# ravenprotocol/ravnest

Measured on AMD Instinct MI355X. Metric: samples/sec (whole node), BERT-base MLM pretraining, higher is better.
Workload: dtype bf16; 1 GPU; model=bert-base, global_batch=128, seq_len=512, parallelism=dp1, reduce_factor=4, optimizer=fused_adam

## Files before the change

ravnest_amd/csrc/bindings.cpp:

```cpp
#include <torch/extension.h>

#include <vector>

std::vector<at::Tensor> layernorm_fwd(at::Tensor x, at::Tensor w,
                                      at::Tensor b, double eps);
std::vector<at::Tensor> layernorm_bwd(at::Tensor dy, at::Tensor x,
                                      at::Tensor w, at::Tensor mean,
                                      at::Tensor rstd);
std::vector<at::Tensor> layernorm_add_fwd(at::Tensor a, at::Tensor b,
                                          at::Tensor w, at::Tensor bias,
                                          double eps);
at::Tensor bias_gelu_fwd(at::Tensor x, at::Tensor bias);
at::Tensor bias_gelu_bwd(at::Tensor dy, at::Tensor x, at::Tensor bias);
at::Tensor colsum_bf16(at::Tensor x);
std::vector<at::Tensor> bias_gelu_bwd_db(at::Tensor dy, at::Tensor x,
                                         at::Tensor bias);
std::vector<at::Tensor> batchnorm_fwd(at::Tensor x, at::Tensor w,
                                      at::Tensor b, at::Tensor running_mean,
                                      at::Tensor running_var, bool training,
                                      double momentum, double eps);
std::vector<at::Tensor> batchnorm_bwd(at::Tensor dy, at::Tensor x,
                                      at::Tensor w, at::Tensor mean,
                                      at::Tensor rstd);
at::Tensor conv2d_fwd(at::Tensor x, at::Tensor w,
                      c10::optional<at::Tensor> bias, long st, long pad,
                      bool relu);
at::Tensor conv2d_dgrad(at::Tensor dy, at::Tensor w, long N, long H,
                        long W, long st, long pad);
at::Tensor conv2d_wgrad(at::Tensor dy, at::Tensor x, long R, long S,
                        long st, long pad);
std::vector<at::Tensor> mx_quant(at::Tensor x);
std::vector<at::Tensor> gemm_nt_bf16(at::Tensor A2, at::Tensor B,
                                     c10::optional<at::Tensor> bias,
                                     int64_t epi);
at::Tensor gemm_wgrad_bf16(at::Tensor dy, at::Tensor x);
at::Tensor mx_gemm(at::Tensor x, at::Tensor xs, at::Tensor w,
                   at::Tensor ws);
at::Tensor mx_gemm2(at::Tensor xq, at::Tensor xs, at::Tensor wq,
                    at::Tensor ws);
at::Tensor mx_scale_probe(at::Tensor a, at::Tensor b, at::Tensor sa,
                          at::Tensor sb);
at::Tensor softmax_fwd(at::Tensor x);
at::Tensor softmax_bwd(at::Tensor dy, at::Tensor y);
std::vector<at::Tensor> maxpool2d_fwd(at::Tensor x, long K, long S, long P);
at::Tensor maxpool2d_bwd(at::Tensor dy, at::Tensor idx, long H, long W,
                         long K, long S, long P);
at::Tensor avgpool2d_fwd(at::Tensor x, long K, long S, long P,
                         bool include_pad);
at::Tensor avgpool2d_bwd(at::Tensor dy, long H, long W, long K, long S,
                         long P, bool include_pad);
at::Tensor global_avgpool_fwd(at::Tensor x);
at::Tensor global_avgpool_bwd(at::Tensor dy, long H, long W);
std::vector<at::Tensor> emb2_ln_fwd(at::Tensor ids, at::Tensor word,
                                    at::Tensor pos, at::Tensor w,
                                    at::Tensor b, double eps);
at::Tensor emb2_add_fwd(at::Tensor ids, at::Tensor word, at::Tensor pos);
std::vector<at::Tensor> emb2_bwd(at::Tensor dx, at::Tensor ids, long V,
                                 long P);
std::vector<at::Tensor> dropout_fwd(at::Tensor x, double p, int64_t seed,
                                    c10::optional<at::Tensor> seed_buf);
at::Tensor dropout_bwd(at::Tensor dy, at::Tensor mask, double p);
std::vector<at::Tensor> dropout_add_ln_fwd(at::Tensor z, at::Tensor a,
                                           at::Tensor w, at::Tensor bias,
                                           double eps, double p, int64_t seed,
                                           c10::optional<at::Tensor> seed_buf);
std::vector<at::Tensor> dropout_add_ln_bwd(at::Tensor dy, at::Tensor s,
                                           at::Tensor w, at::Tensor mean,
                                           at::Tensor rstd,
                                           at::Tensor maskbits, double p);
std::vector<at::Tensor> ce_fwd(at::Tensor logits, at::Tensor targets,
                               int64_t ignore_index);
at::Tensor ce_bwd(at::Tensor logits, at::Tensor targets, at::Tensor lse,
                  at::Tensor gscale, int64_t ignore_index);
std::tuple<at::Tensor, long, long> adam_build_table(
    std::vector<at::Tensor> ps, std::vector<at::Tensor> gs,
    std::vector<at::Tensor> ms, std::vector<at::Tensor> vs,
    std::vector<at::Tensor> masters);
std::tuple<at::Tensor, long, long> grad_build_table(
    std::vector<at::Tensor> gs);
void grad_sqnorm(at::Tensor table, long nchunks, long esize,
                 at::Tensor partials, long offset);
void grad_norm_finalize(at::Tensor partials, long n, at::Tensor stats,
                        double max_norm,
                        c10::optional<at::Tensor> max_norm_buf);
void scale_mt(at::Tensor table, long nchunks, long esize, at::Tensor gstats);
void fused_adam_graph(at::Tensor table, long nchunks, long esize,
                      at::Tensor lr_buf, double b1, double b2, double eps,
                      double wd, at::Tensor step_buf,
                      c10::optional<at::Tensor> gstats);
void fused_adam_table(at::Tensor table, long nchunks, long esize, double lr,
                      double b1, double b2, double eps, double wd, double bc1,
                      double bc2, c10::optional<at::Tensor> gstats);
void fused_sgd_table(at::Tensor table, long nchunks, long esize, double lr,
                     double momentum, double wd, bool nesterov,
                     c10::optional<at::Tensor> gstats);
void fused_lamb_table(at::Tensor table, long nchunks, long esize,
                      long ntensors, double lr, double b1, double b2,
                      double eps, double wd, double bc1, double bc2,
                      double clamp_trust, c10::optional<at::Tensor> gstats);
void fused_adam(std::vector<at::Tensor> ps, std::vector<at::Tensor> gs,
                std::vector<at::Tensor> ms, std::vector<at::Tensor> vs,
                std::vector<at::Tensor> masters, double lr, double b1,
                double b2, double eps, double wd, double bc1, double bc2);
void fused_sgd(std::vector<at::Tensor> ps, std::vector<at::Tensor> gs,
               std::vector<at::Tensor> bufs, std::vector<at::Tensor> masters,
               double lr, double momentum, double wd, bool nesterov);
void fused_lamb(std::vector<at::Tensor> ps, std::vector<at::Tensor> gs,
                std::vector<at::Tensor> ms, std::vector<at::Tensor> vs,
                std::vector<at::Tensor> masters, double lr, double b1,
                double b2, double eps, double wd, double bc1, double bc2,
                double clamp_trust);
void fused_copy(std::vector<at::Tensor> srcs, std::vector<at::Tensor> dsts);
std::vector<at::Tensor> attn_fwd(at::Tensor q, at::Tensor k, at::Tensor v,
                                 at::Tensor mask, bool causal, double scale);
std::vector<at::Tensor> attn_bwd(at::Tensor q, at::Tensor k, at::Tensor v,
                                 at::Tensor o, at::Tensor dout,
                                 at::Tensor lse, at::Tensor mask, bool causal,
                                 double scale);
std::vector<at::Tensor> attn_fwd_qkv(at::Tensor qkv, at::Tensor mask,
                                     bool causal, double scale,
                                     double pdrop, int64_t dseed,
                                     c10::optional<at::Tensor> seed_buf);
at::Tensor attn_bwd_qkv(at::Tensor qkv, at::Tensor o, at::Tensor dout,
                        at::Tensor lse, at::Tensor mask, bool causal,
                        double scale, double pdrop,
                        c10::optional<at::Tensor> mbits);
at::Tensor mfma_probe(at::Tensor a, at::Tensor b);
at::Tensor tr16_probe();
at::Tensor mfma_mx_probe(at::Tensor a, at::Tensor b, int64_t sa, int64_t sb);

PYBIND11_MODULE(TORCH_EXTENSION_NAME, m) {
  m.def("layernorm_fwd", &layernorm_fwd, "fused LayerNorm fwd (CDNA4)");
  m.def("layernorm_bwd", &layernorm_bwd, "fused LayerNorm bwd (CDNA4)");
  m.def("layernorm_add_fwd", &layernorm_add_fwd,
        "fused residual-add + LayerNorm fwd");
  m.def("bias_gelu_fwd", &bias_gelu_fwd, "fused bias+GELU fwd");
  m.def("bias_gelu_bwd", &bias_gelu_bwd, "fused bias+GELU bwd");
  m.def("colsum_bf16", &colsum_bf16, "column sum bf16 -> fp32");
  m.def("bias_gelu_bwd_db", &bias_gelu_bwd_db,
        "fused bias+GELU bwd with in-pass bias-grad column reduction");
  m.def("batchnorm_fwd", &batchnorm_fwd, "fused BatchNorm2d fwd (NCHW)");
  m.def("batchnorm_bwd", &batchnorm_bwd, "fused BatchNorm2d bwd (NCHW)");
  m.def("dropout_fwd", &dropout_fwd, "philox dropout fwd (replayable)",
        py::arg("x"), py::arg("p"), py::arg("seed"),
        py::arg("seed_buf") = py::none());
  m.def("dropout_bwd", &dropout_bwd, "dropout bwd");
  m.def("dropout_add_ln_fwd", &dropout_add_ln_fwd,
        "fused dropout + residual add + LayerNorm fwd (bf16, bit mask)",
        py::arg("z"), py::arg("a"), py::arg("w"), py::arg("bias"),
        py::arg("eps"), py::arg("p"), py::arg("seed"),
        py::arg("seed_buf") = py::none());
  m.def("dropout_add_ln_bwd", &dropout_add_ln_bwd,
        "fused dropout + residual add + LayerNorm bwd: dx, dz, dw, db");
  m.def("conv2d_fwd", &conv2d_fwd,
        "implicit-GEMM MFMA conv fwd (bf16 NCHW)", py::arg("x"),
        py::arg("w"), py::arg("bias") = py::none(), py::arg("st") = 1,
        py::arg("pad") = 0, py::arg("relu") = false);
  m.def("conv2d_dgrad", &conv2d_dgrad, "implicit-GEMM MFMA conv dgrad");
  m.def("conv2d_wgrad", &conv2d_wgrad, "implicit-GEMM MFMA conv wgrad");
  m.def("gemm_nt_bf16", &gemm_nt_bf16,
        "bf16 MFMA GEMM x @ W^T (256^2 8-phase, fused bias/GELU epilogue)",
        py::arg("a"), py::arg("b"), py::arg("bias") = py::none(),
        py::arg("epi") = 0);
  m.def("gemm_wgrad_bf16", &gemm_wgrad_bf16,
        "split-K wgrad dW = dy^T @ x (tr16 transpose reads, fp32 atomics)");
  m.def("mx_quant", &mx_quant,
        "bf16 -> MX fp8 (e4m3 + per-32 e8m0 scales)");
  m.def("mx_gemm", &mx_gemm, "MX fp8 GEMM: x @ W^T, 32x32x64 scaled MFMA");
  m.def("mx_gemm2", &mx_gemm2,
        "LDS-staged MX fp8 GEMM (256^2 4-phase, scaled 32x32x64 MFMA)");
  m.def("mx_scale_probe", &mx_scale_probe,
        "per-lane scale-byte semantics probe");
  m.def("softmax_fwd", &softmax_fwd, "standalone softmax fwd (last dim)");
  m.def("softmax_bwd", &softmax_bwd, "standalone softmax bwd");
  m.def("maxpool2d_fwd", &maxpool2d_fwd, "MaxPool2d fwd (+argmax idx)");
  m.def("maxpool2d_bwd", &maxpool2d_bwd, "MaxPool2d bwd (gather)");
  m.def("avgpool2d_fwd", &avgpool2d_fwd, "AvgPool2d fwd");
  m.def("avgpool2d_bwd", &avgpool2d_bwd, "AvgPool2d bwd");
  m.def("global_avgpool_fwd", &global_avgpool_fwd,
        "global (adaptive 1x1) avg pool fwd");
  m.def("global_avgpool_bwd", &global_avgpool_bwd, "global avg pool bwd");
  m.def("emb2_ln_fwd", &emb2_ln_fwd,
        "fused word+pos embedding gather + LayerNorm fwd");
  m.def("emb2_add_fwd", &emb2_add_fwd, "fused word+pos embedding gather");
  m.def("emb2_bwd", &emb2_bwd,
        "embedding bwd: dword scatter-add + dpos batch reduction");
  m.def("ce_fwd", &ce_fwd, "fused softmax cross-entropy fwd");
  m.def("ce_bwd", &ce_bwd, "fused softmax cross-entropy bwd");
  m.def("fused_adam", &fused_adam, "multi-tensor Adam");
  m.def("adam_build_table", &adam_build_table,
        "prebuild the device chunk table (graph-capturable Adam)");
  m.def("fused_adam_graph", &fused_adam_graph,
        "multi-tensor Adam with device lr/step buffers (hipGraph mode)",
        py::arg("table"), py::arg("nchunks"), py::arg("esize"),
        py::arg("lr_buf"), py::arg("b1"), py::arg("b2"), py::arg("eps"),
        py::arg("wd"), py::arg("step_buf"), py::arg("gstats") = py::none());
  m.def("mt_build_table", &adam_build_table,
        "prebuild the device chunk table (any fused optimizer)");
  m.def("grad_build_table", &grad_build_table,
        "grads-only device chunk table (clip_grad_norm_)");
  m.def("grad_sqnorm", &grad_sqnorm,
        "multi-tensor per-chunk sum of squared grads -> partials");
  m.def("grad_norm_finalize", &grad_norm_finalize,
        "partials -> [norm, clip coefficient, non-finite count]",
        py::arg("partials"), py::arg("n"), py::arg("stats"),
        py::arg("max_norm"), py::arg("max_norm_buf") = py::none());
  m.def("scale_mt", &scale_mt, "multi-tensor in-place g *= stats[1]");
  m.def("fused_adam_table", &fused_adam_table,
        "multi-tensor Adam from a prebuilt table (+ clip coefficient)",
        py::arg("table"), py::arg("nchunks"), py::arg("esize"),
        py::arg("lr"), py::arg("b1"), py::arg("b2"), py::arg("eps"),
        py::arg("wd"), py::arg("bc1"), py::arg("bc2"),
        py::arg("gstats") = py::none());
  m.def("fused_sgd_table", &fused_sgd_table,
        "multi-tensor SGD from a prebuilt table (+ clip coefficient)",
        py::arg("table"), py::arg("nchunks"), py::arg("esize"),
        py::arg("lr"), py::arg("momentum"), py::arg("wd"),
        py::arg("nesterov"), py::arg("gstats") = py::none());
  m.def("fused_lamb_table", &fused_lamb_table,
        "multi-tensor LAMB from a prebuilt table (+ clip coefficient)",
        py::arg("table"), py::arg("nchunks"), py::arg("esize"),
        py::arg("ntensors"), py::arg("lr"), py::arg("b1"), py::arg("b2"),
        py::arg("eps"), py::arg("wd"), py::arg("bc1"), py::arg("bc2"),
        py::arg("clamp_trust"), py::arg("gstats") = py::none());
  m.def("fused_sgd", &fused_sgd, "multi-tensor SGD+momentum");
  m.def("fused_lamb", &fused_lamb, "multi-tensor LAMB");
  m.def("fused_copy", &fused_copy, "multi-tensor device copy");
  m.def("attn_fwd", &attn_fwd, "flash attention fwd (bf16, MFMA)");
  m.def("attn_bwd", &attn_bwd, "flash attention bwd (bf16, MFMA, D=64)");
  m.def("attn_fwd_qkv", &attn_fwd_qkv,
        py::arg("qkv"), py::arg("mask"), py::arg("causal"),
        py::arg("scale"), py::arg("pdrop") = 0.0, py::arg("dseed") = 0,
        py::arg("seed_buf") = py::none(),
        "flash attention fwd, packed (B,S,3,H,D) qkv -> (B,S,H,D)");
  m.def("attn_bwd_qkv", &attn_bwd_qkv,
        py::arg("qkv"), py::arg("o"), py::arg("dout"), py::arg("lse"),
        py::arg("mask"), py::arg("causal"), py::arg("scale"),
        py::arg("pdrop") = 0.0, py::arg("mbits") = py::none(),
        "flash attention bwd, packed qkv -> dqkv");
  m.def("mfma_probe", &mfma_probe, "32x32x16 bf16 MFMA layout probe");
  m.def("tr16_probe", &tr16_probe, "ds_read_b64_tr_b16 mapping probe");
  m.def("mfma_mx_probe", &mfma_mx_probe,
        "32x32x64 MX-scaled fp8 MFMA layout probe");
}
```

ravnest_amd/csrc/ce_loss.hip:

```cpp
#include <torch/extension.h>
#include <ATen/hip/HIPContext.h>

#include "common.h"

namespace {

template <typename T>
DEVINL float ld(const T* p);
template <>
DEVINL float ld<bf16_t>(const bf16_t* p) { return bf2f(*p); }
template <>
DEVINL float ld<float>(const float* p) { return *p; }

DEVINL void ms_merge(float& m, float& s, float m2, float s2) {
  const float mn = fmaxf(m, m2);
  if (mn == -INFINITY) { m = mn; return; }
  s = s * __expf(m - mn) + s2 * __expf(m2 - mn);
  m = mn;
}

template <typename T>
__global__ void ce_fwd_kernel(const T* __restrict__ logits,
                              const long* __restrict__ targets,
                              float* __restrict__ lse_out,
                              float* __restrict__ loss_accum,
                              int* __restrict__ valid_accum, int V, long N,
                              long ignore_index) {
  __shared__ float scratch_m[16];
  __shared__ float scratch_s[16];
  const long row = blockIdx.x;
  if (row >= N) return;
  const T* lr = logits + row * V;
  const long tgt = targets[row];

  float m = -INFINITY, s = 0.f;
  if constexpr (sizeof(T) == 2) {
    const int nv = V >> 3;
    for (int g = threadIdx.x; g < nv; g += blockDim.x) {
      const bf16x8 v8 = *reinterpret_cast<const bf16x8*>(lr + g * 8);
      float vals[8], vmax = -INFINITY;
#pragma unroll
      for (int j = 0; j < 8; ++j) {
        vals[j] = us2f((unsigned short)v8[j]);
        vmax = fmaxf(vmax, vals[j]);
      }
      float ls = 0.f;
#pragma unroll
      for (int j = 0; j < 8; ++j) ls += __expf(vals[j] - vmax);
      if (vmax > m) {
        s = s * __expf(m - vmax) + ls;
        m = vmax;
      } else {
        s += ls * __expf(vmax - m);
      }
    }
    for (int i = (nv << 3) + threadIdx.x; i < V; i += blockDim.x) {
      const float v = ld(lr + i);
      if (v > m) {
        s = s * __expf(m - v) + 1.f;
        m = v;
      } else {
        s += __expf(v - m);
      }
    }
  } else {
    for (int i = threadIdx.x; i < V; i += blockDim.x) {
      const float v = ld(lr + i);
      if (v > m) {
        s = s * __expf(m - v) + 1.f;
        m = v;
      } else {
        s += __expf(v - m);
      }
    }
  }
#pragma unroll
  for (int off = 32; off > 0; off >>= 1) {
    float m2 = __shfl_down(m, off, WAVE);
    float s2 = __shfl_down(s, off, WAVE);
    ms_merge(m, s, m2, s2);
  }
  {
    const int lane = threadIdx.x & (WAVE - 1);
    const int wid = threadIdx.x / WAVE;
    const int nw = (blockDim.x + WAVE - 1) / WAVE;
    if (lane == 0) {
      scratch_m[wid] = m;
      scratch_s[wid] = s;
    }
    __syncthreads();
    if (wid == 0) {
      m = (threadIdx.x < nw) ? scratch_m[threadIdx.x] : -INFINITY;
      s = (threadIdx.x < nw) ? scratch_s[threadIdx.x] : 0.f;
#pragma unroll
      for (int off = 32; off > 0; off >>= 1) {
        float m2 = __shfl_down(m, off, WAVE);
        float s2 = __shfl_down(s, off, WAVE);
        ms_merge(m, s, m2, s2);
      }
      if (threadIdx.x == 0) {
        scratch_m[0] = m;
        scratch_s[0] = s;
      }
    }
    __syncthreads();
    m = scratch_m[0];
    s = scratch_s[0];
  }
  const float lse = m + __logf(s);

  if (threadIdx.x == 0) {
    lse_out[row] = lse;
    if (tgt != ignore_index) {
      atomicAdd(loss_accum, lse - ld(lr + tgt));
      atomicAdd(valid_accum, 1);
    }
  }
}

template <typename T>
__global__ void ce_bwd_kernel(const T* __restrict__ logits,
                              const long* __restrict__ targets,
                              const float* __restrict__ lse,
                              const float* __restrict__ gscale,
                              T* __restrict__ dlogits, int V, long N,
                              long ignore_index) {
  const long row = blockIdx.x;
  if (row >= N) return;
  const T* lr = logits + row * V;
  T* dr = dlogits + row * V;
  const long tgt = targets[row];
  const float g = gscale[0];
  const float l = lse[row];
  if (tgt == ignore_index) {
    for (int i = threadIdx.x; i < V; i += blockDim.x) {
      if constexpr (sizeof(T) == 2)
        dr[i] = f2bf(0.f);
      else
        dr[i] = 0.f;
    }
    return;
  }
  if constexpr (sizeof(T) == 2) {
    const int nv = V >> 3;
    for (int gi = threadIdx.x; gi < nv; gi += blockDim.x) {
      const bf16x8 v8 = *reinterpret_cast<const bf16x8*>(lr + gi * 8);
      bf16x8 o;
#pragma unroll
      for (int j = 0; j < 8; ++j) {
        const int i = gi * 8 + j;
        float p = __expf(us2f((unsigned short)v8[j]) - l);
        o[j] = (short)f2us((p - (i == (int)tgt ? 1.f : 0.f)) * g);
      }
      *reinterpret_cast<bf16x8*>(dr + gi * 8) = o;
    }
    for (int i = (nv << 3) + threadIdx.x; i < V; i += blockDim.x) {
      float p = __expf(ld(lr + i) - l);
      dr[i] = f2bf((p - (i == (int)tgt ? 1.f : 0.f)) * g);
    }
  } else {
    for (int i = threadIdx.x; i < V; i += blockDim.x) {
      float p = __expf(ld(lr + i) - l);
      dr[i] = (p - (i == (int)tgt ? 1.f : 0.f)) * g;
    }
  }
}

}

std::vector<at::Tensor> ce_fwd(at::Tensor logits, at::Tensor targets,
                               int64_t ignore_index) {
  TORCH_CHECK(logits.is_cuda() && logits.is_contiguous());
  TORCH_CHECK(logits.dim() == 2);
  TORCH_CHECK(targets.scalar_type() == at::kLong);
  const long N = logits.size(0);
  const int V = logits.size(1);
  auto lse = at::empty({N}, logits.options().dtype(at::kFloat));
  auto loss = at::zeros({1}, logits.options().dtype(at::kFloat));
  auto nvalid = at::zeros({1}, logits.options().dtype(at::kInt));
  auto stream = c10::hip::getCurrentHIPStreamMasqueradingAsCUDA().stream();
  dim3 block(256);
  dim3 grid(N);
  if (logits.scalar_type() == at::kBFloat16) {
    hipLaunchKernelGGL((ce_fwd_kernel<bf16_t>), grid, block, 0, stream,
                       reinterpret_cast<const bf16_t*>(logits.data_ptr()),
                       targets.data_ptr<long>(), lse.data_ptr<float>(),
                       loss.data_ptr<float>(), nvalid.data_ptr<int>(), V, N,
                       ignore_index);
  } else {
    hipLaunchKernelGGL((ce_fwd_kernel<float>), grid, block, 0, stream,
                       logits.data_ptr<float>(), targets.data_ptr<long>(),
                       lse.data_ptr<float>(), loss.data_ptr<float>(),
                       nvalid.data_ptr<int>(), V, N, ignore_index);
  }
  HIP_CHECK_LAST();
  return {loss.squeeze(0), lse, nvalid.squeeze(0)};
}

at::Tensor ce_bwd(at::Tensor logits, at::Tensor targets, at::Tensor lse,
                  at::Tensor gscale, int64_t ignore_index) {
  TORCH_CHECK(logits.is_cuda() && logits.is_contiguous());
  const long N = logits.size(0);
  const int V = logits.size(1);
  auto dlogits = at::empty_like(logits);
  auto gs = gscale.to(at::kFloat).reshape({1}).contiguous();
  auto stream = c10::hip::getCurrentHIPStreamMasqueradingAsCUDA().stream();
  dim3 block(256);
  dim3 grid(N);
  if (logits.scalar_type() == at::kBFloat16) {
    hipLaunchKernelGGL((ce_bwd_kernel<bf16_t>), grid, block, 0, stream,
                       reinterpret_cast<const bf16_t*>(logits.data_ptr()),
                       targets.data_ptr<long>(), lse.data_ptr<float>(),
                       gs.data_ptr<float>(),
                       reinterpret_cast<bf16_t*>(dlogits.data_ptr()), V, N,
                       ignore_index);
  } else {
    hipLaunchKernelGGL((ce_bwd_kernel<float>), grid, block, 0, stream,
                       logits.data_ptr<float>(), targets.data_ptr<long>(),
                       lse.data_ptr<float>(), gs.data_ptr<float>(),
                       dlogits.data_ptr<float>(), V, N, ignore_index);
  }
  HIP_CHECK_LAST();
  return dlogits;
}
```

ravnest_amd/csrc/gemm.hip:

```cpp
#include <torch/extension.h>
#include <ATen/hip/HIPContext.h>

#include "common.h"

typedef __bf16 bf16x8v __attribute__((ext_vector_type(8)));
typedef unsigned short u16x4 __attribute__((ext_vector_type(4)));

#define LDS_V8(p)                                            \
  *reinterpret_cast<__attribute__((address_space(3))) const  \
                        bf16x8v*>(                           \
      (__attribute__((address_space(3))) const void*)(p))

namespace {

constexpr int BM = 256, BN = 256, BK = 64;
constexpr int HALF_BYTES = 128 * BK * 2;
constexpr int TILE_BYTES = 2 * HALF_BYTES;
constexpr int BUF_BYTES = 2 * TILE_BYTES;

DEVINL float gelu_f(float x) {
  const float k = 0.7978845608028654f;
  const float t = __expf(2.f * k * (x + 0.044715f * x * x * x));
  return x * t / (t + 1.f);
}

DEVINL unsigned stage_off(long ld, long gR0, long gRmax, int i) {
  const int tid = threadIdx.x;
  const int p = i * 8192 + (tid >> 6) * 1024 + (tid & 63) * 16;
  const int rr = p >> 7;
  const int cb = (p & 127) ^ (((p >> 8) & 7) << 4);
  long g = gR0 + rr;
  if (g > gRmax) g = gRmax;
  return (unsigned)(g * ld * 2 + cb);
}

DEVINL int frag_off(int rr, int kc, int lane) {
  const int cb = ((lane >> 4) << 4) + (kc << 6);
  const int p = (rr << 7) + cb;
  return p ^ (((p >> 8) & 7) << 4);
}

template <int EPI>
__global__ __launch_bounds__(512, 2) void gemm_nt_kernel(
    const bf16_t* __restrict__ A, const bf16_t* __restrict__ B,
    const bf16_t* __restrict__ bias, bf16_t* __restrict__ C,
    bf16_t* __restrict__ H, long M, long N, long K, int MT, int NTb,
    int tpb) {
  __shared__ char smem[2 * BUF_BYTES];

  const int nwg = MT * NTb;
  int bid = blockIdx.x, wg;
  if ((nwg & 7) == 0) {
    wg = (bid & 7) * (nwg >> 3) + (bid >> 3);
  } else {
    const int q = nwg >> 3, r = nwg & 7, x = bid & 7, lin = bid >> 3;
    wg = (x < r ? x * (q + 1) : r * (q + 1) + (x - r) * q) + lin;
  }
  constexpr int GM = 8;
  const int group = wg / (GM * NTb);
  const int lid = wg % (GM * NTb);
  const int gsz = min(GM, MT - group * GM);
  const int bm = group * GM + lid % gsz;
  const int bn0 = (lid / gsz) * tpb;

  const int tid = threadIdx.x;
  const int lane = tid & 63;
  const int wid = tid >> 6;
  const int wm = wid >> 2, wn = wid & 3;

  const long mBase = (long)bm * BM;
  const long nBase = (long)bn0 * BN;
  const int nKT = (int)(K / BK);
  const unsigned SJ = (unsigned)(BN * K * 2);

  unsigned sp[4][2];
  unsigned capB[2];
#pragma unroll
  for (int i = 0; i < 2; ++i) {
    sp[0][i] = stage_off(K, mBase, M - 1, i);
    sp[1][i] = stage_off(K, mBase + 128, M - 1, i);
    sp[2][i] = stage_off(K, nBase, N - 1, i);
    sp[3][i] = stage_off(K, nBase + 128, N - 1, i);
    capB[i] = stage_off(K, 0, 0, i) + (unsigned)((N - 1) * K * 2);
  }
  const int slo[4] = {0, HALF_BYTES, TILE_BYTES, TILE_BYTES + HALF_BYTES};
  const int wbase = (threadIdx.x >> 6) * 1024;
  auto stage = [&](int jj, int tt, int kind) {
    if (jj >= tpb) {
      jj = tpb - 1;
      tt = nKT - 1;
    }
    const unsigned off = (unsigned)tt * (BK * 2);
    const int b = (jj * nKT + tt) & 1;
    char* const lb = smem + b * BUF_BYTES + slo[kind] + wbase;
    const char* const base =
        reinterpret_cast<const char*>(kind >= 2 ? B : A);
#pragma unroll
    for (int i = 0; i < 2; ++i) {
      unsigned o = sp[kind][i];
      if (kind >= 2) {
        o += (unsigned)jj * SJ;
        if (o > capB[i]) o = capB[i];
      }
      __builtin_amdgcn_global_load_lds(
          (const __attribute__((address_space(1))) void*)(base + o + off),
          (__attribute__((address_space(3))) void*)(lb + i * 8192),
          16, 0, 0);
    }
  };
  auto norm = [&](int j, int t, int dt, int& jj, int& tt) {
    tt = t + dt;
    jj = j;
    if (tt >= nKT) {
      tt -= nKT;
      ++jj;
    }
  };

  stage(0, 0, 0); stage(0, 0, 2); stage(0, 0, 3); stage(0, 0, 1);
  stage(0, 1, 2); stage(0, 1, 3); stage(0, 1, 0);
  asm volatile("s_waitcnt vmcnt(6)" ::: "memory");
  __builtin_amdgcn_s_barrier();

  const int l15 = lane & 15;

  bf16x8v aF[4][2], bF[4][2];

  for (int j = 0; j < tpb; ++j) {
  f32x4 acc[8][4];
#pragma unroll
  for (int m = 0; m < 8; ++m)
#pragma unroll
    for (int n = 0; n < 4; ++n) acc[m][n] = f32x4{0.f, 0.f, 0.f, 0.f};

  for (int t = 0; t < nKT; ++t) {
    const int b = (j * nKT + t) & 1;
    int jj, tt;
    char* const aH0 = smem + b * BUF_BYTES + wm * HALF_BYTES;
    char* const bH =
        smem + b * BUF_BYTES + TILE_BYTES + (wn >> 1) * HALF_BYTES;
    const int bRow0 = (wn & 1) * 64;

#pragma unroll
    for (int nf = 0; nf < 2; ++nf)
#pragma unroll
      for (int kc = 0; kc < 2; ++kc)
        bF[nf][kc] = LDS_V8(bH + frag_off(bRow0 + nf * 16 + l15, kc, lane));
#pragma unroll
    for (int mf = 0; mf < 4; ++mf)
#pragma unroll
      for (int kc = 0; kc < 2; ++kc)
        aF[mf][kc] = LDS_V8(aH0 + frag_off(mf * 16 + l15, kc, lane));
    norm(j, t, 1, jj, tt);
    stage(jj, tt, 1);
    asm volatile("s_waitcnt lgkmcnt(8)" ::: "memory");
    __builtin_amdgcn_s_setprio(1);
#pragma unroll
    for (int mf = 0; mf < 4; ++mf)
#pragma unroll
      for (int nf = 0; nf < 2; ++nf)
#pragma unroll
        for (int kc = 0; kc < 2; ++kc)
          acc[mf][nf] = __builtin_amdgcn_mfma_f32_16x16x32_bf16(
              bF[nf][kc], aF[mf][kc], acc[mf][nf], 0, 0, 0);
    __builtin_amdgcn_s_setprio(0);
    __builtin_amdgcn_s_barrier();

#pragma unroll
    for (int nf = 2; nf < 4; ++nf)
#pragma unroll
      for (int kc = 0; kc < 2; ++kc)
        bF[nf][kc] = LDS_V8(bH + frag_off(bRow0 + nf * 16 + l15, kc, lane));
    __builtin_amdgcn_s_setprio(1);
#pragma unroll
    for (int mf = 0; mf < 4; ++mf)
#pragma unroll
      for (int nf = 2; nf < 4; ++nf)
#pragma unroll
        for (int kc = 0; kc < 2; ++kc)
          acc[mf][nf] = __builtin_amdgcn_mfma_f32_16x16x32_bf16(
              bF[nf][kc], aF[mf][kc], acc[mf][nf], 0, 0, 0);
    __builtin_amdgcn_s_setprio(0);
    __builtin_amdgcn_s_barrier();

#pragma unroll
    for (int mf = 0; mf < 4; ++mf)
#pragma unroll
      for (int kc = 0; kc < 2; ++kc)
        aF[mf][kc] = LDS_V8(aH0 + frag_off(64 + mf * 16 + l15, kc, lane));
    norm(j, t, 2, jj, tt);
    stage(jj, tt, 2);
    __builtin_amdgcn_s_setprio(1);
#pragma unroll
    for (int mf = 0; mf < 4; ++mf)
#pragma unroll
      for (int nf = 0; nf < 2; ++nf)
#pragma unroll
        for (int kc = 0; kc < 2; ++kc)
          acc[4 + mf][nf] = __builtin_amdgcn_mfma_f32_16x16x32_bf16(
              bF[nf][kc], aF[mf][kc], acc[4 + mf][nf], 0, 0, 0);
    __builtin_amdgcn_s_setprio(0);
    __builtin_amdgcn_s_barrier();

    stage(jj, tt, 3);
    stage(jj, tt, 0);
    __builtin_amdgcn_s_setprio(1);
#pragma unroll
    for (int mf = 0; mf < 4; ++mf)
#pragma unroll
      for (int nf = 2; nf < 4; ++nf)
#pragma unroll
        for (int kc = 0; kc < 2; ++kc)
          acc[4 + mf][nf] = __builtin_amdgcn_mfma_f32_16x16x32_bf16(
              bF[nf][kc], aF[mf][kc], acc[4 + mf][nf], 0, 0, 0);
    __builtin_amdgcn_s_setprio(0);
    asm volatile("s_waitcnt vmcnt(6)" ::: "memory");
    __builtin_amdgcn_s_barrier();
  }

  const long mRow0 = mBase + wm * 128 + l15;
  const long nCol0 = nBase + (long)j * BN + wn * 64 + ((lane >> 4) << 2);
  auto epilogue = [&](auto interior) {
#pragma unroll
    for (int mf = 0; mf < 8; ++mf) {
      const long m = mRow0 + mf * 16;
      if constexpr (!interior.value) {
        if (m >= M) continue;
      }
#pragma unroll
      for (int nf = 0; nf < 4; ++nf) {
        const long n = nCol0 + nf * 16;
        bool full = true;
        if constexpr (!interior.value) {
          if (n >= N) continue;
          full = (n + 4 <= N);
        }
        float v0 = acc[mf][nf][0], v1 = acc[mf][nf][1];
        float v2 = acc[mf][nf][2], v3 = acc[mf][nf][3];
        if (EPI >= 1) {
          if (full) {
            const u16x4 bb = *reinterpret_cast<const u16x4*>(bias + n);
            v0 += us2f(bb[0]); v1 += us2f(bb[1]);
            v2 += us2f(bb[2]); v3 += us2f(bb[3]);
          } else {
            v0 += bf2f(bias[n]);
            if (n + 1 < N) v1 += bf2f(bias[n + 1]);
            if (n + 2 < N) v2 += bf2f(bias[n + 2]);
          }
        }
        if (EPI == 2) {
          u16x4 h{f2us(v0), f2us(v1), f2us(v2), f2us(v3)};
          if (full) {
            *reinterpret_cast<u16x4*>(H + m * N + n) = h;
          } else {
            for (int v = 0; v < 4; ++v)
              if (n + v < N) H[m * N + n + v] = f2bf(us2f(h[v]));
          }
          v0 = gelu_f(v0); v1 = gelu_f(v1);
          v2 = gelu_f(v2); v3 = gelu_f(v3);
        }
        const u16x4 o{f2us(v0), f2us(v1), f2us(v2), f2us(v3)};
        if (full) {
          *reinterpret_cast<u16x4*>(C + m * N + n) = o;
        } else {
          for (int v = 0; v < 4; ++v)
            if (n + v < N) C[m * N + n + v] = f2bf(us2f(o[v]));
        }
      }
    }
  };
  if (mRow0 + 7 * 16 < M && nCol0 + 3 * 16 + 4 <= N)
    epilogue(std::true_type{});
  else
    epilogue(std::false_type{});
  }
  asm volatile("s_waitcnt vmcnt(0)" ::: "memory");
}

}

std::vector<at::Tensor> gemm_nt_bf16(at::Tensor A2, at::Tensor B,
                                     c10::optional<at::Tensor> bias,
                                     int64_t epi) {
  TORCH_CHECK(A2.is_cuda() && A2.scalar_type() == at::kBFloat16 &&
              A2.is_contiguous() && A2.dim() == 2);
  TORCH_CHECK(B.is_cuda() && B.scalar_type() == at::kBFloat16 &&
              B.is_contiguous() && B.dim() == 2);
  const long M = A2.size(0), K = A2.size(1), N = B.size(0);
  TORCH_CHECK(B.size(1) == K, "gemm_nt_bf16: K mismatch");
  TORCH_CHECK(K % BK == 0 && K >= 2 * BK,
              "gemm_nt_bf16: K % 64 == 0 and K >= 128 required");
  TORCH_CHECK(A2.numel() * 2 < (1ll << 32) && B.numel() * 2 < (1ll << 32),
              "gemm_nt_bf16: operands must be < 4 GiB (32-bit staging "
              "offsets)");
  TORCH_CHECK(epi == 0 || bias.has_value(), "bias required for epi>=1");
  const bf16_t* bp = nullptr;
  if (bias.has_value()) {
    TORCH_CHECK(bias->is_contiguous() &&
                bias->scalar_type() == at::kBFloat16 && bias->numel() == N);
    bp = reinterpret_cast<const bf16_t*>(bias->data_ptr());
  }
  auto C = at::empty({M, N}, A2.options());
  at::Tensor Hp;
  bf16_t* hp = nullptr;
  if (epi == 2) {
    Hp = at::empty({M, N}, A2.options());
    hp = reinterpret_cast<bf16_t*>(Hp.data_ptr());
  }
  const int MT = (int)((M + BM - 1) / BM), NT = (int)((N + BN - 1) / BN);
  int tpb = 1;
  for (int cand : {8, 6, 4, 3, 2}) {
    if (NT % cand == 0 && (long)MT * (NT / cand) >= 512) {
      tpb = cand;
      break;
    }
  }
  const int NTb = NT / tpb;
  auto stream = c10::hip::getCurrentHIPStreamMasqueradingAsCUDA().stream();
  dim3 grid((unsigned)(MT * NTb)), block(512);
  auto* a = reinterpret_cast<const bf16_t*>(A2.data_ptr());
  auto* b = reinterpret_cast<const bf16_t*>(B.data_ptr());
  auto* c = reinterpret_cast<bf16_t*>(C.data_ptr());
  switch (epi) {
    case 0:
      hipLaunchKernelGGL((gemm_nt_kernel<0>), grid, block, 0, stream, a, b,
                         bp, c, hp, M, N, K, MT, NTb, tpb);
      break;
    case 1:
      hipLaunchKernelGGL((gemm_nt_kernel<1>), grid, block, 0, stream, a, b,
                         bp, c, hp, M, N, K, MT, NTb, tpb);
      break;
    default:
      hipLaunchKernelGGL((gemm_nt_kernel<2>), grid, block, 0, stream, a, b,
                         bp, c, hp, M, N, K, MT, NTb, tpb);
  }
  HIP_CHECK_LAST();
  if (epi == 2) return {C, Hp};
  return {C};
}
```

ravnest_amd/csrc/gemm_wgrad.hip:

```cpp
#include <torch/extension.h>
#include <ATen/hip/HIPContext.h>

#include "common.h"

typedef __bf16 bf16x4v __attribute__((ext_vector_type(4)));
typedef __bf16 bf16x8v __attribute__((ext_vector_type(8)));
typedef short s16x8 __attribute__((ext_vector_type(8)));

#define DS_TR16(p)                                   \
  __builtin_amdgcn_ds_read_tr16_b64_v4bf16(          \
      (__attribute__((address_space(3))) bf16x4v*)(  \
          (__attribute__((address_space(3))) void*)(p)))

namespace {

constexpr int BN = 128, BK = 128, BM = 64;
constexpr int ROWB = 256;
constexpr int DY_BYTES = BM * ROWB;
constexpr int PAIR_BYTES = 2 * DY_BYTES;

DEVINL int swz(int row, int cb) { return cb ^ ((row & 7) << 5); }

template <bool TAIL>
__global__ __launch_bounds__(256, 2) void wgrad_kernel(
    const bf16_t* __restrict__ DY, const bf16_t* __restrict__ X,
    float* __restrict__ WS, long M, long N, long K, int NT, int KT,
    int splitk, long mTilesPer) {
  __shared__ char smem[2 * PAIR_BYTES];

  const int ntiles = NT * KT;
  const int nwg = ntiles * splitk;
  int bid = blockIdx.x, wg;
  if ((nwg & 7) == 0) {
    wg = (bid & 7) * (nwg >> 3) + (bid >> 3);
  } else {
    const int q = nwg >> 3, r = nwg & 7, x = bid & 7, lin = bid >> 3;
    wg = (x < r ? x * (q + 1) : r * (q + 1) + (x - r) * q) + lin;
  }
  const int tile = wg / splitk, slice = wg % splitk;
  const int bn = tile % NT, bk = tile / NT;
  const long n0 = (long)bn * BN, k0 = (long)bk * BK;
  const bool is_tail = (n0 + BN > N) || (k0 + BK > K);
  if (TAIL != is_tail) return;
  const long mt0 = slice * mTilesPer;
  const long mt1 = min(mt0 + mTilesPer, M / BM);
  if (mt0 >= mt1) return;

  const int tid = threadIdx.x;
  const int lane = tid & 63;
  const int wid = tid >> 6;
  const int wn = wid >> 1, wk = wid & 1;

  auto img = [&](int b, int op) {
    return smem + b * PAIR_BYTES + op * DY_BYTES;
  };

  long srcOff[8];
  int dstOff[8];
  int shiftv[8], validv[8];
#pragma unroll
  for (int i = 0; i < 8; ++i) {
    const int o = i * 4096 + wid * 1024 + lane * 16;
    const int op = o >= DY_BYTES;
    const int lo = op ? o - DY_BYTES : o;
    const int row = lo >> 8;
    const int cb = swz(row, lo & 255);
    const long cols = op ? K : N;
    const long cbase = op ? k0 : n0;
    long c = cbase + cb / 2;
    int sh = 0, va = 8;
    if (TAIL && c + 8 > cols) {
      const long cl = max(0l, cols - 8);
      sh = (int)(c - cl);
      va = (int)max(0l, min(8l, cols - c));
      c = cl;
    }
    srcOff[i] = ((long)row * cols + c) * 2;
    dstOff[i] = o;
    shiftv[i] = sh;
    validv[i] = va;
  }
  const long dyStep = (long)BM * N * 2, xStep = (long)BM * K * 2;

  auto stage_glds = [&](long mt, int b) {
#pragma unroll
    for (int i = 0; i < 8; ++i) {
      const int op = dstOff[i] >= DY_BYTES;
      const char* src = reinterpret_cast<const char*>(op ? X : DY) +
                        srcOff[i] + mt * (op ? xStep : dyStep);
      __builtin_amdgcn_global_load_lds(
          (const __attribute__((address_space(1))) void*)src,
          (__attribute__((address_space(3))) void*)(
              smem + b * PAIR_BYTES + (dstOff[i] - lane * 16)),
          16, 0, 0);
    }
  };

  s16x8 stg[8];
  auto issue_loads = [&](long mt) {
#pragma unroll
    for (int i = 0; i < 8; ++i) {
      const int op = dstOff[i] >= DY_BYTES;
      const char* s = reinterpret_cast<const char*>(op ? X : DY) +
                      srcOff[i] + mt * (op ? xStep : dyStep);
      stg[i] = *reinterpret_cast<const s16x8*>(s);
    }
  };
  auto write_stage = [&](int b) {
#pragma unroll
    for (int i = 0; i < 8; ++i) {
      s16x8 v = stg[i];
      if (shiftv[i] | (validv[i] ^ 8)) {
        s16x8 w;
        for (int j = 0; j < 8; ++j)
          w[j] = (j < validv[i]) ? v[j + shiftv[i]] : short(0);
        v = w;
      }
      *reinterpret_cast<s16x8*>(smem + b * PAIR_BYTES + dstOff[i]) = v;
    }
  };

  const int q4 = lane & 15, g = lane >> 4;
  auto tr_off = [&](int mc, int r, int colwin) {
    const int row = mc * 32 + g * 8 + r * 4 + (q4 >> 2);
    const int cb = (colwin + 4 * (q4 & 3)) * 2;
    return row * ROWB + swz(row, cb);
  };

  f32x4 acc[4][4];
#pragma unroll
  for (int a = 0; a < 4; ++a)
#pragma unroll
    for (int b = 0; b < 4; ++b) acc[a][b] = f32x4{0.f, 0.f, 0.f, 0.f};

  if (TAIL) {
    issue_loads(mt0);
    write_stage(0);
    __syncthreads();
  } else {
    stage_glds(mt0, 0);
    asm volatile("s_waitcnt vmcnt(0)" ::: "memory");
    __builtin_amdgcn_s_barrier();
  }

  for (long mt = mt0; mt < mt1; ++mt) {
    const int b = (int)((mt - mt0) & 1);
    if (mt + 1 < mt1) {
      if (TAIL)
        issue_loads(mt + 1);
      else
        stage_glds(mt + 1, b ^ 1);
    }

    bf16x8v aF[4][2], bF[4][2];
#pragma unroll
    for (int nf = 0; nf < 4; ++nf)
#pragma unroll
      for (int mc = 0; mc < 2; ++mc) {
        bf16x4v lo = DS_TR16(img(b, 0) + tr_off(mc, 0, wn * 64 + nf * 16));
        bf16x4v hi = DS_TR16(img(b, 0) + tr_off(mc, 1, wn * 64 + nf * 16));
        bf16x8v f;
        f[0] = lo[0]; f[1] = lo[1]; f[2] = lo[2]; f[3] = lo[3];
        f[4] = hi[0]; f[5] = hi[1]; f[6] = hi[2]; f[7] = hi[3];
        aF[nf][mc] = f;
      }
#pragma unroll
    for (int kf = 0; kf < 4; ++kf)
#pragma unroll
      for (int mc = 0; mc < 2; ++mc) {
        bf16x4v lo = DS_TR16(img(b, 1) + tr_off(mc, 0, wk * 64 + kf * 16));
        bf16x4v hi = DS_TR16(img(b, 1) + tr_off(mc, 1, wk * 64 + kf * 16));
        bf16x8v f;
        f[0] = lo[0]; f[1] = lo[1]; f[2] = lo[2]; f[3] = lo[3];
        f[4] = hi[0]; f[5] = hi[1]; f[6] = hi[2]; f[7] = hi[3];
        bF[kf][mc] = f;
      }

    __builtin_amdgcn_s_setprio(1);
#pragma unroll
    for (int mc = 0; mc < 2; ++mc)
#pragma unroll
      for (int nf = 0; nf < 4; ++nf)
#pragma unroll
        for (int kf = 0; kf < 4; ++kf)
          acc[nf][kf] = __builtin_amdgcn_mfma_f32_16x16x32_bf16(
              aF[nf][mc], bF[kf][mc], acc[nf][kf], 0, 0, 0);
    __builtin_amdgcn_s_setprio(0);

    if (TAIL) {
      if (mt + 1 < mt1) write_stage(b ^ 1);
      __syncthreads();
    } else {
      asm volatile("s_waitcnt vmcnt(0)" ::: "memory");
      __builtin_amdgcn_s_barrier();
    }
  }

#pragma unroll
  for (int nf = 0; nf < 4; ++nf)
#pragma unroll
    for (int kf = 0; kf < 4; ++kf) {
      const long k = k0 + wk * 64 + kf * 16 + (lane & 15);
      if (k >= K) continue;
#pragma unroll
      for (int v = 0; v < 4; ++v) {
        const long n = n0 + wn * 64 + nf * 16 + ((lane >> 4) << 2) + v;
        if (n < N) atomicAdd(WS + n * K + k, acc[nf][kf][v]);
      }
    }
}

}

at::Tensor gemm_wgrad_bf16(at::Tensor dy, at::Tensor x) {
  TORCH_CHECK(dy.is_cuda() && dy.scalar_type() == at::kBFloat16 &&
              dy.is_contiguous() && dy.dim() == 2);
  TORCH_CHECK(x.is_cuda() && x.scalar_type() == at::kBFloat16 &&
              x.is_contiguous() && x.dim() == 2);
  const long M = dy.size(0), N = dy.size(1), K = x.size(1);
  TORCH_CHECK(x.size(0) == M, "gemm_wgrad: M mismatch");
  TORCH_CHECK(M % BM == 0 && M >= 2 * BM,
              "gemm_wgrad: M % 64 == 0 and M >= 128 required");
  TORCH_CHECK(N >= 8 && K >= 8);
  auto ws = at::zeros({N, K}, dy.options().dtype(at::kFloat));
  const int NT = (int)((N + BN - 1) / BN), KT = (int)((K + BK - 1) / BK);
  const long mTiles = M / BM;
  const int ntiles = NT * KT;
  int splitk = (int)std::min<long>(
      mTiles, std::max<long>(1, (1536 + ntiles - 1) / ntiles));
  const long mTilesPer = (mTiles + splitk - 1) / splitk;
  splitk = (int)((mTiles + mTilesPer - 1) / mTilesPer);
  auto stream = c10::hip::getCurrentHIPStreamMasqueradingAsCUDA().stream();
  dim3 grid((unsigned)(ntiles * splitk)), block(256);
  const bool has_tail = (N % BN) || (K % BK);
  hipLaunchKernelGGL((wgrad_kernel<false>), grid, block, 0, stream,
                     reinterpret_cast<const bf16_t*>(dy.data_ptr()),
                     reinterpret_cast<const bf16_t*>(x.data_ptr()),
                     ws.data_ptr<float>(), M, N, K, NT, KT, splitk,
                     mTilesPer);
  if (has_tail)
    hipLaunchKernelGGL((wgrad_kernel<true>), grid, block, 0, stream,
                       reinterpret_cast<const bf16_t*>(dy.data_ptr()),
                       reinterpret_cast<const bf16_t*>(x.data_ptr()),
                       ws.data_ptr<float>(), M, N, K, NT, KT, splitk,
                       mTilesPer);
  HIP_CHECK_LAST();
  return ws;
}
```

ravnest_amd/engine/compute.py:

```python
from __future__ import annotations

import os
import threading
from dataclasses import dataclass

import torch

from ..utils import current_rng_states, restore_rng_states, trace_range


@dataclass
class _FpidRecord:
    version: int
    rng: dict
    args: list
    needs_grad: list
    recomputed_args: list | None = None
    recomputed_outputs: tuple | None = None


class ComputeEngine:
    def __init__(self, model: torch.nn.Module,
                 optimizer: torch.optim.Optimizer | None,
                 device: torch.device,
                 update_frequency: int = 1,
                 criterion=None,
                 loss_filename: str = "losses.txt",
                 amp_dtype: torch.dtype | None = None,
                 versioning: bool = True,
                 max_grad_norm: float | None = None):
        self.model = model
        self.optimizer = optimizer
        self.device = device
        self.update_frequency = max(1, update_frequency)
        self.criterion = criterion
        self.loss_filename = loss_filename
        self.amp_dtype = amp_dtype
        self.versioning = versioning
        self.max_grad_norm = max_grad_norm
        self._clip_external = False
        self._last_norm = None
        if max_grad_norm is not None and optimizer is not None:
            if hasattr(optimizer, "grad_norm_stats"):
                optimizer.max_grad_norm = max_grad_norm
            else:
                self._clip_external = True
        self._graph_step = None
        if (not versioning and device.type == "cuda"
                and self.update_frequency == 1 and criterion is not None
                and os.environ.get("RAVNEST_CUDA_GRAPH", "1") == "1"):
            from .graphstep import GraphedTrainStep
            self._graph_step = GraphedTrainStep(model, criterion, device,
                                                optimizer=optimizer)

        self.pre_step_hook = None

        self.current_version = 0
        self.version_to_param: dict[int, list[torch.Tensor]] = {}
        self.version_refs: dict[int, int] = {}
        self.fpids: dict[int, _FpidRecord] = {}
        self.n_backwards = 0
        self.file_loss = 0.0
        self._recompute_thread: threading.Thread | None = None
        self._lock = threading.Lock()

        self._params = list(self.model.parameters())
        self._snapshot_current()

    def _optimizer_step(self):
        if self._clip_external:
            from ..ops import clip_grad_norm_
            self._last_norm = clip_grad_norm_(self._params,
                                              self.max_grad_norm)
        self.optimizer.step()

    def last_grad_norm(self) -> float | None:
        if self.max_grad_norm is None or self.optimizer is None:
            return None
        if self._clip_external:
            return None if self._last_norm is None \
                else float(self._last_norm)
        stats = self.optimizer.grad_norm_stats()
        return None if stats is None else float(stats[0])

    def _autocast(self):
        if self.amp_dtype is not None and self.device.type == "cuda":
            return torch.autocast("cuda", dtype=self.amp_dtype)
        import contextlib
        return contextlib.nullcontext()

    def _snapshot_current(self):
        if not self.versioning:
            return
        snap = [torch.empty_like(p) for p in self._params]
        self._fast_copy([p.detach() for p in self._params], snap)
        self.version_to_param[self.current_version] = snap
        self.version_refs.setdefault(self.current_version, 0)

    def _fast_copy(self, srcs, dsts):
        if srcs and srcs[0].is_cuda:
            from ..ops import get_ext
            ext = get_ext(required=False)
            if ext is not None:
                ext.fused_copy(srcs, dsts)
                return
        for s, d in zip(srcs, dsts):
            d.copy_(s)

    def latest_state_snapshot(self) -> dict:
        with self._lock:
            if not self.versioning:
                return {"version": self.current_version,
                        "params": [p.detach().clone() for p in self._params]}
            return {
                "version": self.current_version,
                "params": [t.clone() for t in
                           self.version_to_param[self.current_version]],
            }

    def load_param_list(self, params: list[torch.Tensor]):
        with torch.no_grad():
            for p, src in zip(self._params, params):
                p.data.copy_(src.to(p.device))
        self.bump_version()

    def _release_version(self, v: int):
        self.version_refs[v] -= 1
        if self.version_refs[v] == 0 and v != self.current_version:
            del self.version_refs[v]
            del self.version_to_param[v]

    def bump_version(self):
        old = self.current_version
        self.current_version += 1
        if not self.versioning:
            return
        self._snapshot_current()
        if self.version_refs.get(old, 0) == 0:
            self.version_refs.pop(old, None)
            self.version_to_param.pop(old, None)

    def _swap_params_to(self, version: int):
        snap = self.version_to_param[version]
        for p, s in zip(self._params, snap):
            p.data = s

    def _restore_params(self):
        for p, orig in zip(self._params, self._orig_data):
            p.data = orig

    def forward(self, fpid: int, args: list, needs_grad: list) -> tuple:
        self.join_recompute()
        if not self.model.training:
            self.model.train()
        rng = current_rng_states(self.device)
        rec = _FpidRecord(version=self.current_version, rng=rng,
                          args=[a.detach().clone() if torch.is_tensor(a) else a
                                for a in args],
                          needs_grad=list(needs_grad))
        with torch.no_grad(), self._autocast(), trace_range(f"fwd:{fpid}"):
            out = self.model(*args)
        outputs = out if isinstance(out, tuple) else (out,)
        with self._lock:
            self.fpids[fpid] = rec
            self.version_refs[rec.version] = self.version_refs.get(rec.version, 0) + 1
        return outputs

    def _recompute(self, fpid: int):
        rec = self.fpids[fpid]
        if rec.recomputed_outputs is not None:
            return
        args = []
        for a, ng in zip(rec.args, rec.needs_grad):
            if torch.is_tensor(a) and a.is_floating_point():
                a = a.detach().clone().requires_grad_(True) if ng else a
            args.append(a)
        self._orig_data = [p.data for p in self._params]
        self._swap_params_to(rec.version)
        try:
            if not self.model.training:
                self.model.train()
            devices = [self.device] if self.device.type == "cuda" else []
            with torch.random.fork_rng(devices=devices):
                restore_rng_states(rec.rng, self.device)
                with self._autocast():
                    out = self.model(*args)
        finally:
            self._restore_params()
        rec.recomputed_outputs = out if isinstance(out, tuple) else (out,)
        rec.recomputed_args = args

    def join_recompute(self):
        t = self._recompute_thread
        if t is not None and t.is_alive():
            t.join()

    def backward(self, fpid: int, grads_by_out_idx: dict[int, torch.Tensor],
                 speculative_next: bool = True
                 ) -> tuple[list[torch.Tensor | None], bool]:
        self.join_recompute()
        rec = self.fpids[fpid]
        self._recompute(fpid)
        outs, grads = [], []
        for k, g in grads_by_out_idx.items():
            out = rec.recomputed_outputs[k]
            if out.grad_fn is None:
                continue
            outs.append(out)
            grads.append(g.to(out.dtype).to(out.device))
        if outs:
            with trace_range(f"bwd:{fpid}"):
                torch.autograd.backward(outs, grads)

        input_grads: list[torch.Tensor | None] = []
        for a, ng in zip(rec.recomputed_args, rec.needs_grad):
            if ng and torch.is_tensor(a):
                input_grads.append(a.grad if a.grad is not None
                                   else torch.zeros_like(a))
            else:
                input_grads.append(None)

        stepped = self._finish_backward(fpid, rec)
        if speculative_next and (fpid + 1) in self.fpids:
            self._recompute_thread = threading.Thread(
                target=self._recompute, args=(fpid + 1,), daemon=True)
            self._recompute_thread.start()
        return input_grads, stepped

    def _finish_backward(self, fpid: int, rec: _FpidRecord) -> bool:
        with self._lock:
            del self.fpids[fpid]
            self._release_version(rec.version)
        self.n_backwards += 1
        stepped = False
        if self.optimizer is not None and \
                self.n_backwards % self.update_frequency == 0:
            if self.pre_step_hook is not None:
                self.pre_step_hook()
            self._optimizer_step()
            self.optimizer.zero_grad(set_to_none=True)
            self.model.zero_grad(set_to_none=True)
            self.bump_version()
            stepped = True
        return stepped

    def find_loss(self, fpid: int, args: list, needs_grad: list, targets
                  ) -> tuple[list[torch.Tensor | None], bool, float]:
        self.join_recompute()
        if not self.model.training:
            self.model.train()
        if self._graph_step is not None and not any(needs_grad) and \
                self.amp_dtype is None:
            if self.pre_step_hook is not None:
                self.pre_step_hook()
            loss_t = self._graph_step.run(args, targets)
            if loss_t is not None:
                return self._finish_graphed_step(args, loss_t)
        if self._graph_step is not None and self._graph_step.graphs:
            self.model.zero_grad(set_to_none=True)
        live_args = []
        for a, ng in zip(args, needs_grad):
            if ng and torch.is_tensor(a) and a.is_floating_point():
                a = a.detach().clone().requires_grad_(True)
            live_args.append(a)
        with self._autocast():
            out = self.model(*live_args)
            loss = self.criterion(out, targets)
        loss.backward()
        loss_val = float(loss.detach())
        self.file_loss += loss_val

        input_grads: list[torch.Tensor | None] = []
        for a, ng in zip(live_args, needs_grad):
            if ng and torch.is_tensor(a):
                input_grads.append(a.grad if a.grad is not None
                                   else torch.zeros_like(a))
            else:
                input_grads.append(None)

        self.n_backwards += 1
        stepped = False
        if self.optimizer is not None and \
                self.n_backwards % self.update_frequency == 0:
            if self.pre_step_hook is not None:
                self.pre_step_hook()
            self._optimizer_step()
            self.optimizer.zero_grad(set_to_none=True)
            self.model.zero_grad(set_to_none=True)
            self.bump_version()
            stepped = True
            if self.loss_filename:
                with open(self.loss_filename, "a") as f:
                    f.write(f"{round(self.file_loss, 4)}\n")
            self.file_loss = 0.0
        return input_grads, stepped, loss_val

    def _finish_graphed_step(self, args, loss_t):
        self.n_backwards += 1
        stepped = False
        if self._graph_step.opt_captured:
            self.optimizer.bump_host_steps()
            stepped = True
        elif self.optimizer is not None:
            self._optimizer_step()
            stepped = True
        loss_val = float(loss_t)
        self.file_loss += loss_val
        if stepped:
            if self.loss_filename:
                with open(self.loss_filename, "a") as f:
                    f.write(f"{round(self.file_loss, 4)}\n")
            self.file_loss = 0.0
        return [None] * len(args), stepped, loss_val

    def no_grad_forward(self, args: list) -> tuple:
        self.join_recompute()
        self.model.eval()
        with torch.no_grad(), self._autocast():
            out = self.model(*args)
        return out if isinstance(out, tuple) else (out,)
```

ravnest_amd/engine/graphstep.py:

```python
from __future__ import annotations

import torch

from ..ops import rng


def _sig(tensors):
    return tuple((tuple(t.shape), t.dtype) for t in tensors)


class GraphedTrainStep:

    WARMUP = 3

    def __init__(self, model, criterion, device, optimizer=None):
        self.model = model
        self.criterion = criterion
        self.device = device
        import os
        use_opt = os.environ.get("RAVNEST_GRAPH_OPT", "0") == "1"
        self.optimizer = (optimizer if use_opt and
                          hasattr(optimizer, "graph_step") else None)
        self.opt_captured = False
        self.graphs = {}
        self.pool = None
        self.failed = False

    def run(self, args, targets):
        if self.failed or self.device.type != "cuda":
            return None
        if not all(torch.is_tensor(a) for a in args) or \
                not torch.is_tensor(targets):
            return None
        arg_ts = list(args)
        tgt_ts = [targets]
        key = (_sig(arg_ts), _sig(tgt_ts))
        entry = self.graphs.get(key)
        if entry is None:
            try:
                entry = self._capture(arg_ts, tgt_ts)
            except Exception:
                self.failed = True
                self.model.zero_grad(set_to_none=True)
                return None
            self.graphs[key] = entry
        graph, s_args, s_tgts, s_loss, grad_refs = entry
        if self.opt_captured:
            self.optimizer.sync_lr()
        for dst, src in zip(s_args, arg_ts):
            dst.copy_(src, non_blocking=True)
        for dst, src in zip(s_tgts, tgt_ts):
            dst.copy_(src, non_blocking=True)
        graph.replay()
        for param, gref in grad_refs:
            param.grad = gref
        return s_loss

    def _capture(self, arg_ts, tgt_ts):
        s_args = [t.clone() for t in arg_ts]
        s_tgts = [t.clone() for t in tgt_ts]
        self.model.train()
        rng.device_seed_counter(self.device)

        if self.optimizer is not None and not self.opt_captured:
            self.opt_captured = self.optimizer.enable_graph_capture(
                self.device)

        def step(with_opt=False, stable_grads=None):
            rng.bump_seed_counter(self.device)
            if with_opt:
                torch._foreach_zero_(stable_grads)
            out = self.model(*s_args)
            loss = self.criterion(out, s_tgts[0])
            loss.backward()
            if with_opt:
                self.optimizer.graph_step()
            return loss

        side = torch.cuda.Stream(self.device)
        side.wait_stream(torch.cuda.current_stream(self.device))
        with torch.cuda.stream(side):
            for _ in range(self.WARMUP):
                step()
        torch.cuda.current_stream(self.device).wait_stream(side)
        self.model.zero_grad(set_to_none=True)
        stable_grads = None
        if self.opt_captured:
            stable_grads = self.optimizer._graph.get("grads")
            if stable_grads is None:
                stable_grads = self.optimizer.build_graph_table()

        graph = torch.cuda.CUDAGraph()
        if self.pool is None:
            with torch.cuda.graph(graph):
                s_loss = step(self.opt_captured, stable_grads)
            self.pool = graph.pool()
        else:
            with torch.cuda.graph(graph, pool=self.pool):
                s_loss = step(self.opt_captured, stable_grads)
        grad_refs = [(p, p.grad) for p in self.model.parameters()
                     if p.grad is not None]
        return graph, s_args, s_tgts, s_loss, grad_refs
```

ravnest_amd/models/bert.py:

```python
from __future__ import annotations

import torch
import torch.nn as nn

from ..ops import embedding_ln
from ..ops import (AttentionCoreQKV, Dropout, DropoutAddLayerNorm,
                   FusedLayerNorm, GELU, LinearGelu)
from ..ops.linear import make_linear


class BertConfig:
    def __init__(self, vocab_size=30522, hidden=768, layers=12, heads=12,
                 intermediate=3072, max_seq=512, type_vocab=2,
                 dropout=0.1, layer_norm_eps=1e-12):
        self.vocab_size = vocab_size
        self.hidden = hidden
        self.layers = layers
        self.heads = heads
        self.intermediate = intermediate
        self.max_seq = max_seq
        self.type_vocab = type_vocab
        self.dropout = dropout
        self.layer_norm_eps = layer_norm_eps

    @classmethod
    def base(cls, **kw):
        return cls(**kw)

    @classmethod
    def tiny(cls, **kw):
        d = dict(vocab_size=1024, hidden=128, layers=2, heads=2,
                 intermediate=256, max_seq=64)
        d.update(kw)
        return cls(**d)


class BertEmbeddings(nn.Module):
    _is_leaf_module = True

    def __init__(self, cfg: BertConfig):
        super().__init__()
        self.word = nn.Embedding(cfg.vocab_size, cfg.hidden)
        self.position = nn.Embedding(cfg.max_seq, cfg.hidden)
        self.ln = FusedLayerNorm(cfg.hidden, cfg.layer_norm_eps)
        self.drop = Dropout(cfg.dropout)
        self.register_buffer(
            "pos_ids", torch.arange(cfg.max_seq).unsqueeze(0),
            persistent=False)

    def forward(self, input_ids):
        if input_ids.is_cuda and self.word.weight.dtype == torch.bfloat16:
            y = embedding_ln(input_ids, self.word.weight,
                             self.position.weight, self.ln.weight,
                             self.ln.bias, self.ln.eps)
            return self.drop(y)
        S = input_ids.size(1)
        x = self.word(input_ids) + self.position(self.pos_ids[:, :S])
        return self.drop(self.ln(x))


class BertSelfAttention(nn.Module):

    def __init__(self, cfg: BertConfig):
        super().__init__()
        import os
        self.heads = cfg.heads
        self.head_dim = cfg.hidden // cfg.heads
        self.qkv = make_linear(cfg.hidden, 3 * cfg.hidden)
        exact = os.environ.get("RAVNEST_EXACT_ATTN_DROPOUT", "0") == "1"
        self.core = AttentionCoreQKV(
            causal=False, prob_dropout=cfg.dropout if exact else 0.0)
        self.out = make_linear(cfg.hidden, cfg.hidden)

    def forward(self, x, mask):
        qkv = self.qkv(x).unflatten(-1, (3, self.heads, self.head_dim))
        o = self.core(qkv, mask)
        return self.out(o)


class BertLayer(nn.Module):
    def __init__(self, cfg: BertConfig):
        super().__init__()
        self.attn = BertSelfAttention(cfg)
        self.ln1 = DropoutAddLayerNorm(cfg.hidden, cfg.layer_norm_eps,
                                       cfg.dropout)
        self.mlp_in = LinearGelu(cfg.hidden, cfg.intermediate)
        self.mlp_out = make_linear(cfg.intermediate, cfg.hidden)
        self.ln2 = DropoutAddLayerNorm(cfg.hidden, cfg.layer_norm_eps,
                                       cfg.dropout)

    def forward(self, x, mask):
        x = self.ln1(x, self.attn(x, mask))
        x = self.ln2(x, self.mlp_out(self.mlp_in(x)))
        return x


class BertMLMHead(nn.Module):
    def __init__(self, cfg: BertConfig):
        super().__init__()
        self.dense = make_linear(cfg.hidden, cfg.hidden)
        self.act = GELU()
        self.ln = FusedLayerNorm(cfg.hidden, cfg.layer_norm_eps)
        self.decoder = make_linear(cfg.hidden, cfg.vocab_size)

    def forward(self, x):
        return self.decoder(self.ln(self.act(self.dense(x))))


class BertForMLM(nn.Module):

    def __init__(self, cfg: BertConfig | None = None):
        super().__init__()
        self.cfg = cfg or BertConfig.base()
        self.embeddings = BertEmbeddings(self.cfg)
        self.layers = nn.ModuleList(
            [BertLayer(self.cfg) for _ in range(self.cfg.layers)])
        self.head = BertMLMHead(self.cfg)
        self.apply(self._init)

    @staticmethod
    def _init(m):
        from ..ops import Linear as _OpsLinear
        if isinstance(m, (nn.Linear, _OpsLinear)):
            nn.init.normal_(m.weight, std=0.02)
            if m.bias is not None:
                nn.init.zeros_(m.bias)
        elif isinstance(m, nn.Embedding):
            nn.init.normal_(m.weight, std=0.02)

    def forward(self, input_ids, attention_mask):
        m = (1.0 - attention_mask.to(torch.float32)) * -10000.0
        m = m.unsqueeze(1).unsqueeze(2)
        x = self.embeddings(input_ids)
        for layer in self.layers:
            x = layer(x, m)
        return self.head(x)
```

ravnest_amd/ops/__init__.py:

```python
from ._ext import get_ext, has_ext
from .layernorm import (FusedLayerNorm, AddLayerNorm, layer_norm, add_layer_norm)
from .activation import (GELU, LinearGelu, Softmax, gelu, bias_gelu,
                         softmax)
from .dropout import Dropout, dropout
from .dropout_ln import DropoutAddLayerNorm, dropout_add_layer_norm
from .attention import (AttentionCore, AttentionCoreQKV, attention, attention_qkv)
from .losses import CrossEntropyLoss, cross_entropy
from .optim import FusedAdam, FusedSGD, FusedLAMB, clip_grad_norm_
from .batchnorm import FusedBatchNorm2d
from .linear import Linear
from .conv import Conv1x1, conv2d_mfma
from .embedding import embedding_ln, embedding_add
from .pool import MaxPool2d, AvgPool2d, AdaptiveAvgPool2d
from .mx import MXLinear, mx_linear

__all__ = [
    "get_ext", "has_ext",
    "FusedLayerNorm", "AddLayerNorm", "layer_norm", "add_layer_norm",
    "GELU", "LinearGelu", "Softmax", "gelu", "bias_gelu", "softmax",
    "Dropout", "dropout",
    "DropoutAddLayerNorm", "dropout_add_layer_norm",
    "AttentionCore", "AttentionCoreQKV", "attention", "attention_qkv",
    "CrossEntropyLoss", "cross_entropy",
    "FusedAdam", "FusedSGD", "FusedLAMB", "clip_grad_norm_",
    "FusedBatchNorm2d", "Linear", "Conv1x1", "conv2d_mfma",
    "embedding_ln", "embedding_add",
    "MaxPool2d", "AvgPool2d", "AdaptiveAvgPool2d",
    "MXLinear", "mx_linear",
]
```

Before: 1630 samples/s.

## Compute MLM decoder GEMM and cross-entropy only on non-ignored token rows

```diff
diff --git a/ravnest_amd/csrc/bindings.cpp b/ravnest_amd/csrc/bindings.cpp
--- a/ravnest_amd/csrc/bindings.cpp
+++ b/ravnest_amd/csrc/bindings.cpp
@@ -72,6 +72,13 @@
                                int64_t ignore_index);
 at::Tensor ce_bwd(at::Tensor logits, at::Tensor targets, at::Tensor lse,
                   at::Tensor gscale, int64_t ignore_index);
+std::vector<at::Tensor> mlm_head_fwd(at::Tensor h, at::Tensor W,
+                                     at::Tensor b, at::Tensor targets,
+                                     int64_t ignore_index);
+std::vector<at::Tensor> mlm_head_bwd(at::Tensor dloss, at::Tensor logits_c,
+                                     at::Tensor lse, at::Tensor hc,
+                                     at::Tensor tc, at::Tensor pos,
+                                     at::Tensor count, at::Tensor W);
 std::tuple<at::Tensor, long, long> adam_build_table(
     std::vector<at::Tensor> ps, std::vector<at::Tensor> gs,
     std::vector<at::Tensor> ms, std::vector<at::Tensor> vs,
@@ -187,6 +194,11 @@
         "embedding bwd: dword scatter-add + dpos batch reduction");
   m.def("ce_fwd", &ce_fwd, "fused softmax cross-entropy fwd");
   m.def("ce_bwd", &ce_bwd, "fused softmax cross-entropy bwd");
+  m.def("mlm_head_fwd", &mlm_head_fwd,
+        "sparse MLM head fwd: decoder GEMM + CE on the non-ignored rows "
+        "(device-side live count, graph-capturable)");
+  m.def("mlm_head_bwd", &mlm_head_bwd,
+        "sparse MLM head bwd: dh, dW, db (consumes the saved logits)");
   m.def("fused_adam", &fused_adam, "multi-tensor Adam");
   m.def("adam_build_table", &adam_build_table,
         "prebuild the device chunk table (graph-capturable Adam)");
diff --git a/ravnest_amd/csrc/ce_loss.hip b/ravnest_amd/csrc/ce_loss.hip
--- a/ravnest_amd/csrc/ce_loss.hip
+++ b/ravnest_amd/csrc/ce_loss.hip
@@ -17,6 +17,86 @@
   if (mn == -INFINITY) { m = mn; return; }
   s = s * __expf(m - mn) + s2 * __expf(m2 - mn);
   m = mn;
+}
+
+template <typename T>
+DEVINL float row_lse(const T* __restrict__ lr, int V, float* scratch_m,
+                     float* scratch_s) {
+  float m = -INFINITY, s = 0.f;
+  if constexpr (sizeof(T) == 2) {
+    const int nv = V >> 3;
+    for (int g = threadIdx.x; g < nv; g += blockDim.x) {
+      const bf16x8 v8 = *reinterpret_cast<const bf16x8*>(lr + g * 8);
+      float vals[8], vmax = -INFINITY;
+#pragma unroll
+      for (int j = 0; j < 8; ++j) {
+        vals[j] = us2f((unsigned short)v8[j]);
+        vmax = fmaxf(vmax, vals[j]);
+      }
+      float ls = 0.f;
+#pragma unroll
+      for (int j = 0; j < 8; ++j) ls += __expf(vals[j] - vmax);
+      if (vmax > m) {
+        s = s * __expf(m - vmax) + ls;
+        m = vmax;
+      } else {
+        s += ls * __expf(vmax - m);
+      }
+    }
+    for (int i = (nv << 3) + threadIdx.x; i < V; i += blockDim.x) {
+      const float v = ld(lr + i);
+      if (v > m) {
+        s = s * __expf(m - v) + 1.f;
+        m = v;
+      } else {
+        s += __expf(v - m);
+      }
+    }
+  } else {
+    for (int i = threadIdx.x; i < V; i += blockDim.x) {
+      const float v = ld(lr + i);
+      if (v > m) {
+        s = s * __expf(m - v) + 1.f;
+        m = v;
+      } else {
+        s += __expf(v - m);
+      }
+    }
+  }
+#pragma unroll
+  for (int off = 32; off > 0; off >>= 1) {
+    float m2 = __shfl_down(m, off, WAVE);
+    float s2 = __shfl_down(s, off, WAVE);
+    ms_merge(m, s, m2, s2);
+  }
+  {
+    const int lane = threadIdx.x & (WAVE - 1);
+    const int wid = threadIdx.x / WAVE;
+    const int nw = (blockDim.x + WAVE - 1) / WAVE;
+    if (lane == 0) {
+      scratch_m[wid] = m;
+      scratch_s[wid] = s;
+    }
+    __syncthreads();
+    if (wid == 0) {
+      m = (threadIdx.x < nw) ? scratch_m[threadIdx.x] : -INFINITY;
+      s = (threadIdx.x < nw) ? scratch_s[threadIdx.x] : 0.f;
+#pragma unroll
+      for (int off = 32; off > 0; off >>= 1) {
+        float m2 = __shfl_down(m, off, WAVE);
+        float s2 = __shfl_down(s, off, WAVE);
+        ms_merge(m, s, m2, s2);
+      }
+      if (threadIdx.x == 0) {
+        scratch_m[0] = m;
+        scratch_s[0] = s;
+      }
+    }
+    __syncthreads();
+    m = scratch_m[0];
+    s = scratch_s[0];
+  }
+  return m + __logf(s);
 }
 
 template <typename T>
@@ -33,81 +113,7 @@
   const T* lr = logits + row * V;
   const long tgt = targets[row];
 
-  float m = -INFINITY, s = 0.f;
-  if constexpr (sizeof(T) == 2) {
-    const int nv = V >> 3;
-    for (int g = threadIdx.x; g < nv; g += blockDim.x) {
-      const bf16x8 v8 = *reinterpret_cast<const bf16x8*>(lr + g * 8);
-      float vals[8], vmax = -INFINITY;
-#pragma unroll
-      for (int j = 0; j < 8; ++j) {
-        vals[j] = us2f((unsigned short)v8[j]);
-        vmax = fmaxf(vmax, vals[j]);
-      }
-      float ls = 0.f;
-#pragma unroll
-      for (int j = 0; j < 8; ++j) ls += __expf(vals[j] - vmax);
-      if (vmax > m) {
-        s = s * __expf(m - vmax) + ls;
-        m = vmax;
-      } else {
-        s += ls * __expf(vmax - m);
-      }
-    }
-    for (int i = (nv << 3) + threadIdx.x; i < V; i += blockDim.x) {
-      const float v = ld(lr + i);
-      if (v > m) {
-        s = s * __expf(m - v) + 1.f;
-        m = v;
-      } else {
-        s += __expf(v - m);
-      }
-    }
-  } else {
-    for (int i = threadIdx.x; i < V; i += blockDim.x) {
-      const float v = ld(lr + i);
-      if (v > m) {
-        s = s * __expf(m - v) + 1.f;
-        m = v;
-      } else {
-        s += __expf(v - m);
-      }
-    }
-  }
-#pragma unroll
-  for (int off = 32; off > 0; off >>= 1) {
-    float m2 = __shfl_down(m, off, WAVE);
-    float s2 = __shfl_down(s, off, WAVE);
-    ms_merge(m, s, m2, s2);
-  }
-  {
-    const int lane = threadIdx.x & (WAVE - 1);
-    const int wid = threadIdx.x / WAVE;
-    const int nw = (blockDim.x + WAVE - 1) / WAVE;
-    if (lane == 0) {
-      scratch_m[wid] = m;
-      scratch_s[wid] = s;
-    }
-    __syncthreads();
-    if (wid == 0) {
-      m = (threadIdx.x < nw) ? scratch_m[threadIdx.x] : -INFINITY;
-      s = (threadIdx.x < nw) ? scratch_s[threadIdx.x] : 0.f;
-#pragma unroll
-      for (int off = 32; off > 0; off >>= 1) {
-        float m2 = __shfl_down(m, off, WAVE);
-        float s2 = __shfl_down(s, off, WAVE);
-        ms_merge(m, s, m2, s2);
-      }
-      if (threadIdx.x == 0) {
-        scratch_m[0] = m;
-        scratch_s[0] = s;
-      }
-    }
-    __syncthreads();
-    m = scratch_m[0];
-    s = scratch_s[0];
-  }
-  const float lse = m + __logf(s);
+  const float lse = row_lse(lr, V, scratch_m, scratch_s);
 
   if (threadIdx.x == 0) {
     lse_out[row] = lse;
@@ -163,6 +169,58 @@
       float p = __expf(ld(lr + i) - l);
       dr[i] = (p - (i == (int)tgt ? 1.f : 0.f)) * g;
     }
+  }
+}
+
+__global__ void ce_rows_fwd_kernel(const bf16_t* __restrict__ logits,
+                                   const long* __restrict__ tc,
+                                   const int* __restrict__ count,
+                                   float* __restrict__ lse_out,
+                                   float* __restrict__ loss_accum, int V,
+                                   long ld) {
+  __shared__ float scratch_m[16];
+  __shared__ float scratch_s[16];
+  const long row = blockIdx.x;
+  if (row >= *count) return;
+  const bf16_t* lr = logits + row * ld;
+  const float lse = row_lse(lr, V, scratch_m, scratch_s);
+  if (threadIdx.x == 0) {
+    lse_out[row] = lse;
+    atomicAdd(loss_accum, lse - bf2f(lr[tc[row]]));
+  }
+}
+
+__global__ void ce_rows_bwd_kernel(bf16_t* __restrict__ logits,
+                                   const long* __restrict__ tc,
+                                   const int* __restrict__ count,
+                                   const float* __restrict__ lse,
+                                   const float* __restrict__ dloss, int V,
+                                   long ld) {
+  const long row = blockIdx.x;
+  const int cnt = *count;
+  if (row >= (((long)cnt + 63) & ~63l)) return;
+  bf16_t* dr = logits + row * ld;
+  const int nld = (int)(ld >> 3);
+  if (row >= cnt) {
+    const bf16x8 z = {0, 0, 0, 0, 0, 0, 0, 0};
+    for (int gi = threadIdx.x; gi < nld; gi += blockDim.x)
+      *reinterpret_cast<bf16x8*>(dr + gi * 8) = z;
+    return;
+  }
+  const int tgt = (int)tc[row];
+  const float g = dloss[0] / (float)max(cnt, 1);
+  const float l = lse[row];
+  for (int gi = threadIdx.x; gi < nld; gi += blockDim.x) {
+    const bf16x8 v8 = *reinterpret_cast<const bf16x8*>(dr + gi * 8);
+    bf16x8 o;
+#pragma unroll
+    for (int j = 0; j < 8; ++j) {
+      const int i = gi * 8 + j;
+      const float p = __expf(us2f((unsigned short)v8[j]) - l);
+      const float d = (p - (i == tgt ? 1.f : 0.f)) * g;
+      o[j] = i < V ? (short)f2us(d) : (short)0;
+    }
+    *reinterpret_cast<bf16x8*>(dr + gi * 8) = o;
   }
 }
 
@@ -223,3 +281,45 @@
   HIP_CHECK_LAST();
   return dlogits;
 }
+
+std::vector<at::Tensor> ce_rows_fwd(at::Tensor logits, at::Tensor tc,
+                                    at::Tensor count, int64_t V) {
+  TORCH_CHECK(logits.is_cuda() && logits.is_contiguous() &&
+              logits.dim() == 2 && logits.scalar_type() == at::kBFloat16);
+  TORCH_CHECK(tc.scalar_type() == at::kLong && tc.is_contiguous() &&
+              tc.numel() >= logits.size(0));
+  TORCH_CHECK(count.scalar_type() == at::kInt && count.numel() == 1);
+  const long cap = logits.size(0), ld = logits.size(1);
+  TORCH_CHECK(ld % 8 == 0 && V <= ld && V >= 1);
+  auto lse = at::empty({cap}, logits.options().dtype(at::kFloat));
+  auto loss = at::zeros({1}, logits.options().dtype(at::kFloat));
+  auto stream = c10::hip::getCurrentHIPStreamMasqueradingAsCUDA().stream();
+  hipLaunchKernelGGL(ce_rows_fwd_kernel, dim3(cap), dim3(256), 0, stream,
+                     reinterpret_cast<const bf16_t*>(logits.data_ptr()),
+                     tc.data_ptr<long>(), count.data_ptr<int>(),
+                     lse.data_ptr<float>(), loss.data_ptr<float>(), (int)V,
+                     ld);
+  HIP_CHECK_LAST();
+  return {loss.squeeze(0), lse};
+}
+
+void ce_rows_bwd_(at::Tensor logits, at::Tensor tc, at::Tensor count,
+                  at::Tensor lse, at::Tensor dloss, int64_t V) {
+  TORCH_CHECK(logits.is_cuda() && logits.is_contiguous() &&
+              logits.dim() == 2 && logits.scalar_type() == at::kBFloat16);
+  TORCH_CHECK(tc.scalar_type() == at::kLong && tc.is_contiguous());
+  TORCH_CHECK(count.scalar_type() == at::kInt && count.numel() == 1);
+  TORCH_CHECK(lse.scalar_type() == at::kFloat && lse.is_contiguous() &&
+              lse.numel() >= logits.size(0));
+  TORCH_CHECK(dloss.scalar_type() == at::kFloat && dloss.numel() == 1 &&
+              dloss.is_cuda());
+  const long cap = logits.size(0), ld = logits.size(1);
+  TORCH_CHECK(ld % 8 == 0 && V <= ld && cap % 64 == 0);
+  auto stream = c10::hip::getCurrentHIPStreamMasqueradingAsCUDA().stream();
+  hipLaunchKernelGGL(ce_rows_bwd_kernel, dim3(cap), dim3(256), 0, stream,
+                     reinterpret_cast<bf16_t*>(logits.data_ptr()),
+                     tc.data_ptr<long>(), count.data_ptr<int>(),
+                     lse.data_ptr<float>(), dloss.data_ptr<float>(), (int)V,
+                     ld);
+  HIP_CHECK_LAST();
+}
diff --git a/ravnest_amd/csrc/gemm.hip b/ravnest_amd/csrc/gemm.hip
--- a/ravnest_amd/csrc/gemm.hip
+++ b/ravnest_amd/csrc/gemm.hip
@@ -45,10 +45,16 @@
     const bf16_t* __restrict__ A, const bf16_t* __restrict__ B,
     const bf16_t* __restrict__ bias, bf16_t* __restrict__ C,
     bf16_t* __restrict__ H, long M, long N, long K, int MT, int NTb,
-    int tpb) {
+    int tpb, long ldc, const int* __restrict__ mlimit) {
   __shared__ char smem[2 * BUF_BYTES];
 
+  if (mlimit != nullptr) {
+    const long lim = *mlimit;
+    if (lim < M) M = lim < 0 ? 0 : lim;
+    MT = (int)((M + BM - 1) / BM);
+  }
   const int nwg = MT * NTb;
+  if ((int)blockIdx.x >= nwg) return;
   int bid = blockIdx.x, wg;
   if ((nwg & 7) == 0) {
     wg = (bid & 7) * (nwg >> 3) + (bid >> 3);
@@ -251,20 +257,20 @@
         if (EPI == 2) {
           u16x4 h{f2us(v0), f2us(v1), f2us(v2), f2us(v3)};
           if (full) {
-            *reinterpret_cast<u16x4*>(H + m * N + n) = h;
+            *reinterpret_cast<u16x4*>(H + m * ldc + n) = h;
           } else {
             for (int v = 0; v < 4; ++v)
-              if (n + v < N) H[m * N + n + v] = f2bf(us2f(h[v]));
+              if (n + v < N) H[m * ldc + n + v] = f2bf(us2f(h[v]));
           }
           v0 = gelu_f(v0); v1 = gelu_f(v1);
           v2 = gelu_f(v2); v3 = gelu_f(v3);
         }
         const u16x4 o{f2us(v0), f2us(v1), f2us(v2), f2us(v3)};
         if (full) {
-          *reinterpret_cast<u16x4*>(C + m * N + n) = o;
+          *reinterpret_cast<u16x4*>(C + m * ldc + n) = o;
         } else {
           for (int v = 0; v < 4; ++v)
-            if (n + v < N) C[m * N + n + v] = f2bf(us2f(o[v]));
+            if (n + v < N) C[m * ldc + n + v] = f2bf(us2f(o[v]));
         }
       }
     }
@@ -279,9 +285,10 @@
 
 }
 
-std::vector<at::Tensor> gemm_nt_bf16(at::Tensor A2, at::Tensor B,
-                                     c10::optional<at::Tensor> bias,
-                                     int64_t epi) {
+static void launch_gemm_nt(const at::Tensor& A2, const at::Tensor& B,
+                           const c10::optional<at::Tensor>& bias,
+                           int64_t epi, bf16_t* c, bf16_t* hp, long ldc,
+                           const int* mlimit) {
   TORCH_CHECK(A2.is_cuda() && A2.scalar_type() == at::kBFloat16 &&
               A2.is_contiguous() && A2.dim() == 2);
   TORCH_CHECK(B.is_cuda() && B.scalar_type() == at::kBFloat16 &&
@@ -294,12 +301,50 @@
               "gemm_nt_bf16: operands must be < 4 GiB (32-bit staging "
               "offsets)");
   TORCH_CHECK(epi == 0 || bias.has_value(), "bias required for epi>=1");
+  TORCH_CHECK(ldc == N || (ldc > N && ldc % 4 == 0),
+              "gemm_nt_bf16: ldc must cover N (and keep 8-byte stores "
+              "aligned when padded)");
   const bf16_t* bp = nullptr;
   if (bias.has_value()) {
     TORCH_CHECK(bias->is_contiguous() &&
                 bias->scalar_type() == at::kBFloat16 && bias->numel() == N);
     bp = reinterpret_cast<const bf16_t*>(bias->data_ptr());
   }
+  const int MT = (int)((M + BM - 1) / BM), NT = (int)((N + BN - 1) / BN);
+  int tpb = 1;
+  for (int cand : {8, 6, 4, 3, 2}) {
+    if (mlimit != nullptr && cand > 4) continue;
+    if (NT % cand == 0 && (long)MT * (NT / cand) >= 512) {
+      tpb = cand;
+      break;
+    }
+  }
+  const int NTb = NT / tpb;
+  auto stream = c10::hip::getCurrentHIPStreamMasqueradingAsCUDA().stream();
+  dim3 grid((unsigned)(MT * NTb)), block(512);
+  auto* a = reinterpret_cast<const bf16_t*>(A2.data_ptr());
+  auto* b = reinterpret_cast<const bf16_t*>(B.data_ptr());
+  switch (epi) {
+    case 0:
+      hipLaunchKernelGGL((gemm_nt_kernel<0>), grid, block, 0, stream, a, b,
+                         bp, c, hp, M, N, K, MT, NTb, tpb, ldc, mlimit);
+      break;
+    case 1:
+      hipLaunchKernelGGL((gemm_nt_kernel<1>), grid, block, 0, stream, a, b,
+                         bp, c, hp, M, N, K, MT, NTb, tpb, ldc, mlimit);
+      break;
+    default:
+      hipLaunchKernelGGL((gemm_nt_kernel<2>), grid, block, 0, stream, a, b,
+                         bp, c, hp, M, N, K, MT, NTb, tpb, ldc, mlimit);
+  }
+  HIP_CHECK_LAST();
+}
+
+std::vector<at::Tensor> gemm_nt_bf16(at::Tensor A2, at::Tensor B,
+                                     c10::optional<at::Tensor> bias,
+                                     int64_t epi) {
+  TORCH_CHECK(A2.dim() == 2 && B.dim() == 2);
+  const long M = A2.size(0), N = B.size(0);
   auto C = at::empty({M, N}, A2.options());
   at::Tensor Hp;
   bf16_t* hp = nullptr;
@@ -307,34 +352,21 @@
     Hp = at::empty({M, N}, A2.options());
     hp = reinterpret_cast<bf16_t*>(Hp.data_ptr());
   }
-  const int MT = (int)((M + BM - 1) / BM), NT = (int)((N + BN - 1) / BN);
-  int tpb = 1;
-  for (int cand : {8, 6, 4, 3, 2}) {
-    if (NT % cand == 0 && (long)MT * (NT / cand) >= 512) {
-      tpb = cand;
-      break;
-    }
-  }
-  const int NTb = NT / tpb;
-  auto stream = c10::hip::getCurrentHIPStreamMasqueradingAsCUDA().stream();
-  dim3 grid((unsigned)(MT * NTb)), block(512);
-  auto* a = reinterpret_cast<const bf16_t*>(A2.data_ptr());
-  auto* b = reinterpret_cast<const bf16_t*>(B.data_ptr());
-  auto* c = reinterpret_cast<bf16_t*>(C.data_ptr());
-  switch (epi) {
-    case 0:
-      hipLaunchKernelGGL((gemm_nt_kernel<0>), grid, block, 0, stream, a, b,
-                         bp, c, hp, M, N, K, MT, NTb, tpb);
-      break;
-    case 1:
-      hipLaunchKernelGGL((gemm_nt_kernel<1>), grid, block, 0, stream, a, b,
-                         bp, c, hp, M, N, K, MT, NTb, tpb);
-      break;
-    default:
-      hipLaunchKernelGGL((gemm_nt_kernel<2>), grid, block, 0, stream, a, b,
-                         bp, c, hp, M, N, K, MT, NTb, tpb);
-  }
-  HIP_CHECK_LAST();
+  launch_gemm_nt(A2, B, bias, epi, reinterpret_cast<bf16_t*>(C.data_ptr()),
+                 hp, N, nullptr);
   if (epi == 2) return {C, Hp};
   return {C};
 }
+
+void gemm_nt_bf16_rows(at::Tensor A2, at::Tensor B,
+                       c10::optional<at::Tensor> bias, int64_t epi,
+                       at::Tensor C, at::Tensor row_limit) {
+  TORCH_CHECK(epi == 0 || epi == 1, "gemm_nt_bf16_rows: epi 0 or 1");
+  TORCH_CHECK(C.is_cuda() && C.scalar_type() == at::kBFloat16 &&
+              C.is_contiguous() && C.dim() == 2 &&
+              C.size(0) >= A2.size(0) && C.size(1) >= B.size(0));
+  TORCH_CHECK(row_limit.is_cuda() && row_limit.scalar_type() == at::kInt &&
+              row_limit.numel() == 1);
+  launch_gemm_nt(A2, B, bias, epi, reinterpret_cast<bf16_t*>(C.data_ptr()),
+                 nullptr, C.size(1), row_limit.data_ptr<int>());
+}
diff --git a/ravnest_amd/csrc/gemm_wgrad.hip b/ravnest_amd/csrc/gemm_wgrad.hip
--- a/ravnest_amd/csrc/gemm_wgrad.hip
+++ b/ravnest_amd/csrc/gemm_wgrad.hip
@@ -25,7 +25,7 @@
 __global__ __launch_bounds__(256, 2) void wgrad_kernel(
     const bf16_t* __restrict__ DY, const bf16_t* __restrict__ X,
     float* __restrict__ WS, long M, long N, long K, int NT, int KT,
-    int splitk, long mTilesPer) {
+    int splitk, long mTilesPer, const int* __restrict__ mbound) {
   __shared__ char smem[2 * PAIR_BYTES];
 
   const int ntiles = NT * KT;
@@ -42,8 +42,14 @@
   const long n0 = (long)bn * BN, k0 = (long)bk * BK;
   const bool is_tail = (n0 + BN > N) || (k0 + BK > K);
   if (TAIL != is_tail) return;
+  long mTiles = M / BM;
+  if (mbound != nullptr) {
+    const long bt = ((long)max(*mbound, 0) + BM - 1) / BM;
+    if (bt < mTiles) mTiles = bt;
+    mTilesPer = (mTiles + splitk - 1) / splitk;
+  }
   const long mt0 = slice * mTilesPer;
-  const long mt1 = min(mt0 + mTilesPer, M / BM);
+  const long mt1 = min(mt0 + mTilesPer, mTiles);
   if (mt0 >= mt1) return;
 
   const int tid = threadIdx.x;
@@ -212,7 +218,8 @@
 
 }
 
-at::Tensor gemm_wgrad_bf16(at::Tensor dy, at::Tensor x) {
+static at::Tensor launch_wgrad(const at::Tensor& dy, const at::Tensor& x,
+                               const int* mbound) {
   TORCH_CHECK(dy.is_cuda() && dy.scalar_type() == at::kBFloat16 &&
               dy.is_contiguous() && dy.dim() == 2);
   TORCH_CHECK(x.is_cuda() && x.scalar_type() == at::kBFloat16 &&
@@ -237,13 +244,24 @@
                      reinterpret_cast<const bf16_t*>(dy.data_ptr()),
                      reinterpret_cast<const bf16_t*>(x.data_ptr()),
                      ws.data_ptr<float>(), M, N, K, NT, KT, splitk,
-                     mTilesPer);
+                     mTilesPer, mbound);
   if (has_tail)
     hipLaunchKernelGGL((wgrad_kernel<true>), grid, block, 0, stream,
                        reinterpret_cast<const bf16_t*>(dy.data_ptr()),
                        reinterpret_cast<const bf16_t*>(x.data_ptr()),
                        ws.data_ptr<float>(), M, N, K, NT, KT, splitk,
-                       mTilesPer);
+                       mTilesPer, mbound);
   HIP_CHECK_LAST();
   return ws;
 }
+
+at::Tensor gemm_wgrad_bf16(at::Tensor dy, at::Tensor x) {
+  return launch_wgrad(dy, x, nullptr);
+}
+
+at::Tensor gemm_wgrad_bf16_rows(at::Tensor dy, at::Tensor x,
+                                at::Tensor row_bound) {
+  TORCH_CHECK(row_bound.is_cuda() && row_bound.scalar_type() == at::kInt &&
+              row_bound.numel() == 1);
+  return launch_wgrad(dy, x, row_bound.data_ptr<int>());
+}
diff --git a/ravnest_amd/csrc/mlm_head.hip b/ravnest_amd/csrc/mlm_head.hip
--- /dev/null
+++ b/ravnest_amd/csrc/mlm_head.hip
@@ -0,0 +1,272 @@
+#include <torch/extension.h>
+#include <ATen/hip/HIPContext.h>
+
+#include "common.h"
+
+void gemm_nt_bf16_rows(at::Tensor A2, at::Tensor B,
+                       c10::optional<at::Tensor> bias, int64_t epi,
+                       at::Tensor C, at::Tensor row_limit);
+at::Tensor gemm_wgrad_bf16_rows(at::Tensor dy, at::Tensor x,
+                                at::Tensor row_bound);
+std::vector<at::Tensor> ce_rows_fwd(at::Tensor logits, at::Tensor tc,
+                                    at::Tensor count, int64_t V);
+void ce_rows_bwd_(at::Tensor logits, at::Tensor tc, at::Tensor count,
+                  at::Tensor lse, at::Tensor dloss, int64_t V);
+
+namespace {
+
+constexpr int SCAN_THREADS = 256, SCAN_CHUNKS = 8;
+constexpr int SCAN_ROWS = SCAN_THREADS * SCAN_CHUNKS;
+
+DEVINL int block_sum_int(int v, int* lds) {
+  const int lane = threadIdx.x & (WAVE - 1), wid = threadIdx.x / WAVE;
+#pragma unroll
+  for (int off = 32; off > 0; off >>= 1) v += __shfl_down(v, off, WAVE);
+  if (lane == 0) lds[wid] = v;
+  __syncthreads();
+  int r = 0;
+#pragma unroll
+  for (int w = 0; w < SCAN_THREADS / WAVE; ++w) r += lds[w];
+  __syncthreads();
+  return r;
+}
+
+__global__ __launch_bounds__(SCAN_THREADS) void mlm_count_kernel(
+    const long* __restrict__ targets, long N, long ignore_index,
+    int* __restrict__ blockcnt) {
+  __shared__ int lds[SCAN_THREADS / WAVE];
+  const long r0 = (long)blockIdx.x * SCAN_ROWS;
+  int c = 0;
+#pragma unroll
+  for (int k = 0; k < SCAN_CHUNKS; ++k) {
+    const long i = r0 + k * SCAN_THREADS + threadIdx.x;
+    if (i < N) c += targets[i] != ignore_index;
+  }
+  c = block_sum_int(c, lds);
+  if (threadIdx.x == 0) blockcnt[blockIdx.x] = c;
+}
+
+__global__ __launch_bounds__(SCAN_THREADS) void mlm_scan_kernel(
+    const long* __restrict__ targets, long N, long ignore_index,
+    const int* __restrict__ blockcnt, int* __restrict__ pos,
+    int* __restrict__ idx, int* __restrict__ count) {
+  __shared__ int lds[SCAN_THREADS / WAVE];
+  const int tid = threadIdx.x;
+  const int lane = tid & (WAVE - 1), wid = tid / WAVE;
+  int part = 0;
+  for (int j = tid; j < (int)blockIdx.x; j += SCAN_THREADS)
+    part += blockcnt[j];
+  int run = block_sum_int(part, lds);
+  const long r0 = (long)blockIdx.x * SCAN_ROWS;
+  for (int k = 0; k < SCAN_CHUNKS; ++k) {
+    const long i = r0 + k * SCAN_THREADS + tid;
+    const bool live = i < N && targets[i] != ignore_index;
+    const unsigned long long mask = __ballot(live);
+    const int wpre = __popcll(mask & ((1ull << lane) - 1ull));
+    if (lane == 0) lds[wid] = __popcll(mask);
+    __syncthreads();
+    int off = 0, tot = 0;
+#pragma unroll
+    for (int w = 0; w < SCAN_THREADS / WAVE; ++w) {
+      const int t = lds[w];
+      if (w < wid) off += t;
+      tot += t;
+    }
+    __syncthreads();
+    if (live) {
+      const int p = run + off + wpre;
+      pos[i] = p;
+      idx[p] = (int)i;
+    } else if (i < N) {
+      pos[i] = -1;
+    }
+    run += tot;
+  }
+  if (blockIdx.x == gridDim.x - 1 && tid == 0) count[0] = run;
+}
+
+__global__ void mlm_gather_kernel(const bf16_t* __restrict__ h,
+                                  const long* __restrict__ targets,
+                                  const int* __restrict__ idx,
+                                  const int* __restrict__ count,
+                                  bf16_t* __restrict__ hc,
+                                  long* __restrict__ tc, long cap, int Hd) {
+  const long r = (long)blockIdx.x * (blockDim.x / WAVE) + threadIdx.x / WAVE;
+  const int lane = threadIdx.x & (WAVE - 1);
+  const int cnt = *count;
+  if (r >= cap || r >= (((long)cnt + 63) & ~63l)) return;
+  bf16x8* dst = reinterpret_cast<bf16x8*>(hc + r * Hd);
+  const int nv = Hd >> 3;
+  if (r < cnt) {
+    const long src_row = idx[r];
+    const bf16x8* src = reinterpret_cast<const bf16x8*>(h + src_row * Hd);
+    for (int g = lane; g < nv; g += WAVE) dst[g] = src[g];
+    if (lane == 0) tc[r] = targets[src_row];
+  } else {
+    const bf16x8 z = {0, 0, 0, 0, 0, 0, 0, 0};
+    for (int g = lane; g < nv; g += WAVE) dst[g] = z;
+    if (lane == 0) tc[r] = 0;
+  }
+}
+
+__global__ void mlm_scatter_kernel(const bf16_t* __restrict__ dhc,
+                                   const int* __restrict__ pos,
+                                   bf16_t* __restrict__ dh, long N, int Hd) {
+  const long i = (long)blockIdx.x * (blockDim.x / WAVE) + threadIdx.x / WAVE;
+  const int lane = threadIdx.x & (WAVE - 1);
+  if (i >= N) return;
+  bf16x8* dst = reinterpret_cast<bf16x8*>(dh + i * Hd);
+  const int nv = Hd >> 3;
+  const int p = pos[i];
+  if (p >= 0) {
+    const bf16x8* src = reinterpret_cast<const bf16x8*>(dhc + (long)p * Hd);
+    for (int g = lane; g < nv; g += WAVE) dst[g] = src[g];
+  } else {
+    const bf16x8 z = {0, 0, 0, 0, 0, 0, 0, 0};
+    for (int g = lane; g < nv; g += WAVE) dst[g] = z;
+  }
+}
+
+__global__ __launch_bounds__(256) void mlm_transpose_pad_kernel(
+    const bf16_t* __restrict__ W, bf16_t* __restrict__ Wt, long V, long Vp,
+    int Hd) {
+  __shared__ unsigned short tile[64][65];
+  const long v0 = (long)blockIdx.x * 64;
+  const int h0 = blockIdx.y * 64;
+  const int c = threadIdx.x & 63, r0 = threadIdx.x >> 6;
+  const unsigned short* w = reinterpret_cast<const unsigned short*>(W);
+  unsigned short* wt = reinterpret_cast<unsigned short*>(Wt);
+  for (int r = r0; r < 64; r += 4) {
+    const long v = v0 + r;
+    tile[r][c] = v < V ? w[v * Hd + h0 + c] : (unsigned short)0;
+  }
+  __syncthreads();
+  for (int r = r0; r < 64; r += 4)
+    wt[(long)(h0 + r) * Vp + v0 + c] = tile[c][r];
+}
+
+__global__ void mlm_colsum_kernel(const bf16_t* __restrict__ x,
+                                  const int* __restrict__ count,
+                                  float* __restrict__ out, long ld) {
+  const long col = (long)blockIdx.x * blockDim.x + threadIdx.x;
+  if (col >= ld) return;
+  const long cnt = *count;
+  const long per = (cnt + gridDim.y - 1) / gridDim.y;
+  const long r0 = blockIdx.y * per, r1 = min(cnt, r0 + per);
+  if (r0 >= r1) return;
+  float s = 0.f;
+  long r = r0;
+  for (; r + 8 <= r1; r += 8) {
+    float acc[8];
+#pragma unroll
+    for (int j = 0; j < 8; ++j) acc[j] = bf2f(x[(r + j) * ld + col]);
+#pragma unroll
+    for (int j = 0; j < 8; ++j) s += acc[j];
+  }
+  for (; r < r1; ++r) s += bf2f(x[r * ld + col]);
+  atomicAdd(&out[col], s);
+}
+
+inline long round_up64(long v) { return (v + 63) / 64 * 64; }
+inline long pad_vocab(long v) { return (v + 127) / 128 * 128; }
+
+}
+
+std::vector<at::Tensor> mlm_head_fwd(at::Tensor h, at::Tensor W,
+                                     at::Tensor b, at::Tensor targets,
+                                     int64_t ignore_index) {
+  TORCH_CHECK(h.is_cuda() && h.scalar_type() == at::kBFloat16 &&
+              h.is_contiguous() && h.dim() == 2);
+  TORCH_CHECK(W.is_cuda() && W.scalar_type() == at::kBFloat16 &&
+              W.is_contiguous() && W.dim() == 2 && W.size(1) == h.size(1));
+  TORCH_CHECK(b.is_cuda() && b.scalar_type() == at::kBFloat16 &&
+              b.is_contiguous() && b.numel() == W.size(0));
+  TORCH_CHECK(targets.is_cuda() && targets.scalar_type() == at::kLong &&
+              targets.is_contiguous() && targets.numel() == h.size(0));
+  const long N = h.size(0), Hd = h.size(1), V = W.size(0);
+  TORCH_CHECK(Hd % 64 == 0 && Hd >= 128,
+              "mlm_head: hidden % 64 == 0 and >= 128 required");
+  TORCH_CHECK(N >= 1 && N < (1l << 31));
+  const long cap = std::max(round_up64(N), 128l), Vp = pad_vocab(V);
+  TORCH_CHECK(cap * Vp * 2 < (1ll << 32),
+              "mlm_head: compact logits must stay < 4 GiB");
+  auto stream = c10::hip::getCurrentHIPStreamMasqueradingAsCUDA().stream();
+  auto iopt = h.options().dtype(at::kInt);
+  auto count = at::empty({1}, iopt);
+  auto pos = at::empty({N}, iopt);
+  auto idx = at::empty({cap}, iopt);
+  auto hc = at::empty({cap, Hd}, h.options());
+  auto tc = at::empty({cap}, targets.options());
+  auto logits = at::empty({cap, Vp}, h.options());
+
+  const unsigned sblocks = (unsigned)((N + SCAN_ROWS - 1) / SCAN_ROWS);
+  auto blockcnt = at::empty({(long)sblocks}, iopt);
+  hipLaunchKernelGGL(mlm_count_kernel, dim3(sblocks), dim3(SCAN_THREADS), 0,
+                     stream, targets.data_ptr<long>(), N, (long)ignore_index,
+                     blockcnt.data_ptr<int>());
+  hipLaunchKernelGGL(mlm_scan_kernel, dim3(sblocks), dim3(SCAN_THREADS), 0,
+                     stream, targets.data_ptr<long>(), N, (long)ignore_index,
+                     blockcnt.data_ptr<int>(), pos.data_ptr<int>(),
+                     idx.data_ptr<int>(), count.data_ptr<int>());
+  hipLaunchKernelGGL(mlm_gather_kernel, dim3((unsigned)((cap + 3) / 4)),
+                     dim3(256), 0, stream,
+                     reinterpret_cast<const bf16_t*>(h.data_ptr()),
+                     targets.data_ptr<long>(), idx.data_ptr<int>(),
+                     count.data_ptr<int>(),
+                     reinterpret_cast<bf16_t*>(hc.data_ptr()),
+                     tc.data_ptr<long>(), cap, (int)Hd);
+  HIP_CHECK_LAST();
+  gemm_nt_bf16_rows(hc, W, b, 1, logits, count);
+  auto ce = ce_rows_fwd(logits, tc, count, V);
+  return {ce[0], count, logits, ce[1], hc, tc, pos};
+}
+
+std::vector<at::Tensor> mlm_head_bwd(at::Tensor dloss, at::Tensor logits_c,
+                                     at::Tensor lse, at::Tensor hc,
+                                     at::Tensor tc, at::Tensor pos,
+                                     at::Tensor count, at::Tensor W) {
+  TORCH_CHECK(W.is_cuda() && W.scalar_type() == at::kBFloat16 &&
+              W.is_contiguous() && W.dim() == 2);
+  TORCH_CHECK(pos.scalar_type() == at::kInt && pos.is_contiguous());
+  const long N = pos.numel(), Hd = W.size(1), V = W.size(0);
+  const long cap = logits_c.size(0), Vp = logits_c.size(1);
+  TORCH_CHECK(Vp == pad_vocab(V) && cap >= N && cap % 64 == 0);
+  TORCH_CHECK(hc.dim() == 2 && hc.size(0) == cap && hc.size(1) == Hd &&
+              Hd % 64 == 0);
+  auto stream = c10::hip::getCurrentHIPStreamMasqueradingAsCUDA().stream();
+  auto gs = dloss.to(at::kFloat).reshape({1}).contiguous();
+  ce_rows_bwd_(logits_c, tc, count, lse, gs, V);
+
+  auto Wt = at::empty({Hd, Vp}, W.options());
+  hipLaunchKernelGGL(mlm_transpose_pad_kernel,
+                     dim3((unsigned)(Vp / 64), (unsigned)(Hd / 64)),
+                     dim3(256), 0, stream,
+                     reinterpret_cast<const bf16_t*>(W.data_ptr()),
+                     reinterpret_cast<bf16_t*>(Wt.data_ptr()), V, Vp,
+                     (int)Hd);
+  HIP_CHECK_LAST();
+  auto dhc = at::empty({cap, Hd}, W.options());
+  gemm_nt_bf16_rows(logits_c, Wt, c10::nullopt, 0, dhc, count);
+  auto dh = at::empty({N, Hd}, W.options());
+  hipLaunchKernelGGL(mlm_scatter_kernel, dim3((unsigned)((N + 3) / 4)),
+                     dim3(256), 0, stream,
+                     reinterpret_cast<const bf16_t*>(dhc.data_ptr()),
+                     pos.data_ptr<int>(),
+                     reinterpret_cast<bf16_t*>(dh.data_ptr()), N, (int)Hd);
+  HIP_CHECK_LAST();
+
+  auto dWp = gemm_wgrad_bf16_rows(logits_c, hc, count);
+  auto dW = dWp.narrow(0, 0, V).to(W.scalar_type());
+
+  auto dbp = at::zeros({Vp}, W.options().dtype(at::kFloat));
+  const int col_blocks = (int)((Vp + 255) / 256);
+  const int nchunks = (int)std::min<long>(
+      cap / 64, std::max<long>(1, 8192 / col_blocks));
+  hipLaunchKernelGGL(mlm_colsum_kernel, dim3(col_blocks, nchunks), dim3(256),
+                     0, stream,
+                     reinterpret_cast<const bf16_t*>(logits_c.data_ptr()),
+                     count.data_ptr<int>(), dbp.data_ptr<float>(), Vp);
+  HIP_CHECK_LAST();
+  auto db = dbp.narrow(0, 0, V).to(W.scalar_type());
+  return {dh, dW, db};
+}
diff --git a/ravnest_amd/engine/compute.py b/ravnest_amd/engine/compute.py
--- a/ravnest_amd/engine/compute.py
+++ b/ravnest_amd/engine/compute.py
@@ -7,6 +7,7 @@
 import torch
 
 from ..utils import current_rng_states, restore_rng_states, trace_range
+from .fused_loss import model_loss
 
 
 @dataclass
@@ -264,8 +265,8 @@
                 a = a.detach().clone().requires_grad_(True)
             live_args.append(a)
         with self._autocast():
-            out = self.model(*live_args)
-            loss = self.criterion(out, targets)
+            loss = model_loss(self.model, self.criterion, live_args,
+                              targets)
         loss.backward()
         loss_val = float(loss.detach())
         self.file_loss += loss_val
diff --git a/ravnest_amd/engine/fused_loss.py b/ravnest_amd/engine/fused_loss.py
--- /dev/null
+++ b/ravnest_amd/engine/fused_loss.py
@@ -0,0 +1,13 @@
+from __future__ import annotations
+
+import torch
+
+
+def model_loss(model, criterion, args, targets):
+    fused = getattr(model, "forward_loss", None)
+    if fused is not None and torch.is_tensor(targets) and \
+            all(torch.is_tensor(a) for a in args):
+        loss = fused(*args, targets, criterion)
+        if loss is not None and loss is not NotImplemented:
+            return loss
+    return criterion(model(*args), targets)
diff --git a/ravnest_amd/engine/graphstep.py b/ravnest_amd/engine/graphstep.py
--- a/ravnest_amd/engine/graphstep.py
+++ b/ravnest_amd/engine/graphstep.py
@@ -3,6 +3,7 @@
 import torch
 
 from ..ops import rng
+from .fused_loss import model_loss
 
 
 def _sig(tensors):
@@ -70,8 +71,8 @@
             rng.bump_seed_counter(self.device)
             if with_opt:
                 torch._foreach_zero_(stable_grads)
-            out = self.model(*s_args)
-            loss = self.criterion(out, s_tgts[0])
+            loss = model_loss(self.model, self.criterion, s_args,
+                              s_tgts[0])
             loss.backward()
             if with_opt:
                 self.optimizer.graph_step()
diff --git a/ravnest_amd/models/bert.py b/ravnest_amd/models/bert.py
--- a/ravnest_amd/models/bert.py
+++ b/ravnest_amd/models/bert.py
@@ -103,8 +103,11 @@
         self.ln = FusedLayerNorm(cfg.hidden, cfg.layer_norm_eps)
         self.decoder = make_linear(cfg.hidden, cfg.vocab_size)
 
+    def transform(self, x):
+        return self.ln(self.act(self.dense(x)))
+
     def forward(self, x):
-        return self.decoder(self.ln(self.act(self.dense(x))))
+        return self.decoder(self.transform(x))
 
 
 class BertForMLM(nn.Module):
@@ -128,10 +131,34 @@
         elif isinstance(m, nn.Embedding):
             nn.init.normal_(m.weight, std=0.02)
 
-    def forward(self, input_ids, attention_mask):
+    def _encode(self, input_ids, attention_mask):
         m = (1.0 - attention_mask.to(torch.float32)) * -10000.0
         m = m.unsqueeze(1).unsqueeze(2)
         x = self.embeddings(input_ids)
         for layer in self.layers:
             x = layer(x, m)
-        return self.head(x)
+        return x
+
+    def forward(self, input_ids, attention_mask):
+        return self.head(self._encode(input_ids, attention_mask))
+
+    def forward_loss(self, input_ids, attention_mask, targets, criterion):
+        from ..ops.losses import CrossEntropyLoss
+        from ..ops.mlm_head import (sparse_mlm_head_enabled,
+                                    sparse_mlm_head_loss,
+                                    sparse_mlm_head_supported)
+        dec = self.head.decoder
+        if not (self.training and sparse_mlm_head_enabled()
+                and type(criterion) is CrossEntropyLoss
+                and torch.is_tensor(targets) and input_ids.is_cuda
+                and dec.weight.is_cuda
+                and dec.weight.dtype == torch.bfloat16
+                and not torch.is_autocast_enabled()
+                and targets.numel() == input_ids.numel()):
+            return None
+        if not sparse_mlm_head_supported(dec.weight, dec.bias, targets):
+            return None
+        x = self._encode(input_ids, attention_mask)
+        h = self.head.transform(x)
+        return sparse_mlm_head_loss(h, dec.weight, dec.bias, targets,
+                                    criterion.ignore_index)
diff --git a/ravnest_amd/ops/__init__.py b/ravnest_amd/ops/__init__.py
--- a/ravnest_amd/ops/__init__.py
+++ b/ravnest_amd/ops/__init__.py
@@ -6,6 +6,7 @@
 from .dropout_ln import DropoutAddLayerNorm, dropout_add_layer_norm
 from .attention import (AttentionCore, AttentionCoreQKV, attention, attention_qkv)
 from .losses import CrossEntropyLoss, cross_entropy
+from .mlm_head import sparse_mlm_head_loss
 from .optim import FusedAdam, FusedSGD, FusedLAMB, clip_grad_norm_
 from .batchnorm import FusedBatchNorm2d
 from .linear import Linear
@@ -21,7 +22,7 @@
     "Dropout", "dropout",
     "DropoutAddLayerNorm", "dropout_add_layer_norm",
     "AttentionCore", "AttentionCoreQKV", "attention", "attention_qkv",
-    "CrossEntropyLoss", "cross_entropy",
+    "CrossEntropyLoss", "cross_entropy", "sparse_mlm_head_loss",
     "FusedAdam", "FusedSGD", "FusedLAMB", "clip_grad_norm_",
     "FusedBatchNorm2d", "Linear", "Conv1x1", "conv2d_mfma",
     "embedding_ln", "embedding_add",
diff --git a/ravnest_amd/ops/mlm_head.py b/ravnest_amd/ops/mlm_head.py
--- /dev/null
+++ b/ravnest_amd/ops/mlm_head.py
@@ -0,0 +1,65 @@
+from __future__ import annotations
+
+import os
+
+import torch
+
+from ._ext import get_ext
+
+CALLS = 0
+
+
+def sparse_mlm_head_enabled() -> bool:
+    return os.environ.get("RAVNEST_SPARSE_MLM_HEAD", "1") != "0"
+
+
+def sparse_mlm_head_supported(weight: torch.Tensor, bias, targets) -> bool:
+    if bias is None or not torch.is_tensor(targets):
+        return False
+    hd = weight.shape[1]
+    n = targets.numel()
+    cap = max((n + 63) // 64 * 64, 128)
+    vp = (weight.shape[0] + 127) // 128 * 128
+    return (weight.is_cuda and targets.is_cuda
+            and weight.dtype == torch.bfloat16
+            and bias.dtype == torch.bfloat16
+            and targets.dtype == torch.int64
+            and hd % 64 == 0 and hd >= 128 and vp >= 128
+            and n >= 1
+            and cap * vp * 2 < 2 ** 32)
+
+
+class _SparseMLMHeadFn(torch.autograd.Function):
+    @staticmethod
+    def forward(ctx, h2, weight, bias, targets, ignore_index):
+        ext = get_ext(required=True)
+        (loss_sum, count, logits_c, lse, hc, tc, pos) = ext.mlm_head_fwd(
+            h2, weight, bias, targets, ignore_index)
+        ctx.saved = (logits_c, lse, hc, tc, pos, count)
+        ctx.save_for_backward(weight)
+        return loss_sum / count.clamp(min=1)
+
+    @staticmethod
+    def backward(ctx, dloss):
+        if ctx.saved is None:
+            raise RuntimeError(
+                "sparse_mlm_head_loss: backward ran twice (the saved "
+                "logits are consumed in place)")
+        logits_c, lse, hc, tc, pos, count = ctx.saved
+        ctx.saved = None
+        (weight,) = ctx.saved_tensors
+        ext = get_ext(required=True)
+        dh, dw, db = ext.mlm_head_bwd(dloss, logits_c, lse, hc, tc, pos,
+                                      count, weight)
+        return dh, dw, db, None, None
+
+
+def sparse_mlm_head_loss(h: torch.Tensor, weight: torch.Tensor,
+                         bias: torch.Tensor, targets: torch.Tensor,
+                         ignore_index: int = -100) -> torch.Tensor:
+    global CALLS
+    CALLS += 1
+    h2 = h.reshape(-1, h.shape[-1]).contiguous()
+    t2 = targets.reshape(-1).contiguous()
+    return _SparseMLMHeadFn.apply(h2, weight.contiguous(),
+                                  bias.contiguous(), t2, int(ignore_index))
```

Result: faster. 1831 samples/s, median of 6 (+12.3%).
